# gmarcais/Jellyfish

Measured on AMD Instinct MI355X. Metric: k-mers/sec at k=21 canonical, 150 bp synthetic reads, bit-exact counts, higher is better.
Workload: dtype u64

## Files before the change

include/jfgpu.h:

```cpp
#ifndef JFGPU_H
#define JFGPU_H
#include <stddef.h>
#include <stdint.h>

#ifdef __cplusplus
extern "C" {
#endif

#define JFGPU_ABI_VERSION 1

enum {
  JFGPU_OK = 0,
  JFGPU_E_INVALID = 1,
  JFGPU_E_NO_DEVICE = 2,
  JFGPU_E_ALLOC = 3,
  JFGPU_E_FULL = 4,
  JFGPU_E_HIP = 5,
  JFGPU_E_UNSUPPORTED = 6,
  JFGPU_E_FORMAT = 7,
  JFGPU_E_CORRUPT = 8
};

typedef struct jfgpu_table jfgpu_table;

// ... 16 lines not shown
  uint32_t k, key_len;
  uint32_t canonical;
  uint32_t lsize;
  uint64_t size;
  uint64_t local_size;
  uint32_t shard_bits, shard_id;
  uint32_t val_len;
  uint32_t slot_bytes;
  uint32_t tile_slots;
  uint32_t matrix_identity;
  uint32_t out_counter_len;
  uint32_t max_reprobe;
  uint64_t table_bytes;
} jfgpu_info;

typedef struct jfgpu_stats {
  uint64_t unique;
  uint64_t distinct;
  uint64_t total;
  uint64_t max_count;
  uint64_t occupied;
  uint64_t mers_fed;
} jfgpu_stats;

const char* jfgpu_last_error(void);
int  jfgpu_abi_version(void);
int  jfgpu_device_count(void);

int  jfgpu_create(const jfgpu_params* params, jfgpu_table** out);
void jfgpu_destroy(jfgpu_table* t);
int  jfgpu_get_info(const jfgpu_table* t, jfgpu_info* out);
int  jfgpu_get_matrix(const jfgpu_table* t, uint64_t* columns );
int  jfgpu_clear(jfgpu_table* t);
int  jfgpu_sync(jfgpu_table* t);
int  jfgpu_wait(jfgpu_table* t);

int  jfgpu_count_ascii_dev(jfgpu_table* t, const char* d_bases, size_t n);
int  jfgpu_count_ascii(jfgpu_table* t, const char* bases, size_t n);

int  jfgpu_add_keys_dev(jfgpu_table* t, const uint64_t* d_keys, size_t n, uint64_t val, uint8_t* d_is_new);
int  jfgpu_add_keys(jfgpu_table* t, const uint64_t* keys, size_t n, uint64_t val, uint8_t* is_new);

int  jfgpu_add_key_vals(jfgpu_table* t, const uint64_t* keys, const uint64_t* vals, size_t n);

int  jfgpu_lookup_dev(jfgpu_table* t, const uint64_t* d_keys, size_t n, uint64_t* d_vals, uint8_t* d_found);
int  jfgpu_lookup(jfgpu_table* t, const uint64_t* keys, size_t n, uint64_t* vals, uint8_t* found);

int  jfgpu_partition_ascii_dev(jfgpu_table* t, const char* d_bases, size_t n,
                               uint64_t* d_keys_out, size_t capacity, uint64_t* counts_out);

typedef struct jfgpu_comm jfgpu_comm;
int  jfgpu_comm_unique_id(uint8_t* id128);
int  jfgpu_comm_create(int world, int rank, const uint8_t* id128, int device, jfgpu_comm** out);
int  jfgpu_comm_create_local(int world, int device, jfgpu_comm** out);
void jfgpu_comm_destroy(jfgpu_comm* c);
int  jfgpu_comm_count_ascii_dev(jfgpu_comm* c, jfgpu_table* t, const char* d_bases, size_t n);
int  jfgpu_comm_local_step(jfgpu_comm* c, jfgpu_table** tables, const char* const* d_bases, const size_t* n);
int  jfgpu_comm_finish(jfgpu_comm* c, uint64_t* sent, uint64_t* received);
int  jfgpu_comm_allreduce_u64(jfgpu_comm* c, uint64_t* values, int n, int op);
int  jfgpu_comm_allgather_u64(jfgpu_comm* c, uint64_t mine, uint64_t* all);
int  jfgpu_comm_world(const jfgpu_comm* c, int* world, int* rank);
int  jfgpu_comm_exchange_times(jfgpu_comm* c, double* ms, uint64_t* wire_bytes, size_t cap, size_t* n);

int  jfgpu_stats_compute(jfgpu_table* t, uint64_t lower, uint64_t upper, jfgpu_stats* out);
int  jfgpu_digest(jfgpu_table* t, uint64_t lower, uint64_t upper, uint64_t* out4);
int  jfgpu_histo(jfgpu_table* t, uint64_t base, uint64_t ceil, uint64_t inc, uint64_t* histo, uint64_t nb_buckets);
int  jfgpu_dump_begin(jfgpu_table* t, uint64_t lower, uint64_t upper, uint64_t* n_records, uint32_t* record_bytes);
int  jfgpu_dump_next(jfgpu_table* t, void* out, uint64_t capacity_records, uint64_t* n_read);
int  jfgpu_dump_end(jfgpu_table* t);

typedef struct jfgpu_bloom jfgpu_bloom;
typedef struct jfgpu_bloom_params {
  uint32_t k, canonical;
  uint64_t m;
  uint32_t nb_hashes;
  int32_t  device;
  uint64_t seed;
  const uint64_t* matrix1;
  const uint64_t* matrix2;
} jfgpu_bloom_params;
uint64_t jfgpu_bc_opt_m(double fp, uint64_t n);
uint32_t jfgpu_bc_opt_k(double fp);
int  jfgpu_bc_create(const jfgpu_bloom_params* p, jfgpu_bloom** out);
void jfgpu_bc_destroy(jfgpu_bloom* b);
int  jfgpu_bc_insert_ascii_dev(jfgpu_bloom* b, const char* d_bases, size_t n);
int  jfgpu_bc_insert_ascii(jfgpu_bloom* b, const char* bases, size_t n);
int  jfgpu_bc_sync(jfgpu_bloom* b, uint64_t* mers_fed);
int  jfgpu_bc_clear(jfgpu_bloom* b);
int  jfgpu_bc_get_info(const jfgpu_bloom* b, uint64_t* m, uint32_t* nb_hashes, uint64_t* nb_bytes,
                       uint64_t* matrix1 , uint64_t* matrix2);
int  jfgpu_bc_read(jfgpu_bloom* b, uint8_t* out);
int  jfgpu_bc_load(jfgpu_bloom* b, const uint8_t* data);
int  jfgpu_bc_keys(jfgpu_bloom* b, const uint64_t* keys, size_t n, uint8_t* out, int do_insert);
int  jfgpu_bf_create(const jfgpu_bloom_params* p, jfgpu_bloom** out);
int  jfgpu_bc_set_mode(jfgpu_bloom* b, int mode);
int  jfgpu_bc_reserve(jfgpu_bloom* b, uint64_t workspace_bytes);
int  jfgpu_bc_profile_enable(jfgpu_bloom* b, int on);
int  jfgpu_bc_profile_get(jfgpu_bloom* b, int which, double* ms, uint64_t* launches, uint64_t* units);
int  jfgpu_bc_profile_reset(jfgpu_bloom* b);
int  jfgpu_attach_bloom(jfgpu_table* t, jfgpu_bloom* b);
int  jfgpu_comm_bc_merge(jfgpu_comm* c, jfgpu_bloom* b);
int  jfgpu_comm_bc_merge_local(jfgpu_comm* c, jfgpu_bloom** blooms);

int  jfgpu_set_growth(jfgpu_table* t, int on);

int  jfgpu_reference_matrix(uint32_t lsize, uint32_t key_len, uint64_t* columns);

#define JFGPU_OP_COUNT  0
#define JFGPU_OP_PRIME  1
#define JFGPU_OP_UPDATE 2
int  jfgpu_set_operation(jfgpu_table* t, int op);

int  jfgpu_table_bytes(uint32_t k, uint64_t size, uint64_t* slots, uint64_t* bytes);

int  jfgpu_set_spill(jfgpu_table* t, int (*fn)(void* user), void* user);

int  jfgpu_set_mode(jfgpu_table* t, int mode);
int  jfgpu_reserve(jfgpu_table* t, uint64_t input_bytes);

typedef struct jfgpu_parser jfgpu_parser;
#define JFGPU_PARSE_FASTA    1u
#define JFGPU_PARSE_FASTQ    2u
#define JFGPU_PARSE_CONTINUE 4u
int  jfgpu_parser_create(int device, uint32_t k, jfgpu_parser** out);
void jfgpu_parser_destroy(jfgpu_parser* p);
int  jfgpu_parser_parse_dev(jfgpu_parser* p, const char* d_bytes, size_t n, unsigned flags,
                            const char** d_out, size_t* n_out, uint64_t* n_records);
int  jfgpu_parser_parse(jfgpu_parser* p, const char* bytes, size_t n, unsigned flags,
                        const char** d_out, size_t* n_out, uint64_t* n_records);
int  jfgpu_parser_host_buffer(jfgpu_parser* p, int which, size_t bytes, char** out);
int  jfgpu_parser_upload(jfgpu_parser* p, int which, const char* bytes, size_t n);
int  jfgpu_parser_upload_wait(jfgpu_parser* p, int which);
int  jfgpu_parser_parse_uploaded(jfgpu_parser* p, int which, unsigned flags,
                                 const char** d_out, size_t* n_out, uint64_t* n_records);
int  jfgpu_parser_set_min_quality(jfgpu_parser* p, int min_qual_char);
int  jfgpu_parser_last_ms(jfgpu_parser* p, double* ms);

typedef struct jfgpu_bgzf_block {
  uint64_t c_off, u_off;
  uint32_t c_len, isize, crc32, reserved;
} jfgpu_bgzf_block;
int  jfgpu_bgzf_scan(const void* bytes, size_t n, jfgpu_bgzf_block* out, size_t cap, size_t* n_blocks, size_t* n_used);
int  jfgpu_parser_inflate_uploaded(jfgpu_parser* p, int which, const jfgpu_bgzf_block* blocks, size_t n_blocks,
                                   size_t* stream_len);
int  jfgpu_parser_stream_read(jfgpu_parser* p, size_t offset, size_t n, void* dst);
int  jfgpu_parser_stream_consume(jfgpu_parser* p, size_t n);
int  jfgpu_parser_bam_decode(jfgpu_parser* p, size_t skip, int32_t n_ref, const char** d_out, size_t* n_out,
                             uint64_t* n_records, size_t* n_left);

int  jfgpu_profile_enable(jfgpu_table* t, int on);
int  jfgpu_profile_get(jfgpu_table* t, int which, double* ms, uint64_t* launches, uint64_t* units);
int  jfgpu_profile_reset(jfgpu_table* t);
int  jfgpu_profile_spans(jfgpu_table* t, int* which, double* ms, size_t cap, size_t* n);
#define JFGPU_N_COUNTERS 16
int  jfgpu_get_counters(jfgpu_table* t, uint64_t* out, uint32_t n);
int  jfgpu_gen_reads_dev(jfgpu_table* t, char* d_out, uint64_t first_read, uint64_t n_reads, uint32_t read_len, uint64_t seed);
int  jfgpu_gen_genome_reads_dev(jfgpu_table* t, char* d_out, uint64_t first_read, uint64_t n_reads, uint32_t read_len,
                                uint64_t genome_len, double substitution_rate, uint64_t seed);
int  jfgpu_gups(jfgpu_table* t, uint64_t n_updates, int mode, double* updates_per_s);
int  jfgpu_malloc_host(size_t bytes, void** out);
int  jfgpu_free_host(void* p);
int  jfgpu_malloc_dev(jfgpu_table* t, size_t bytes, void** out);
int  jfgpu_free_dev(jfgpu_table* t, void* p);
int  jfgpu_memcpy_h2d(jfgpu_table* t, void* d_dst, const void* src, size_t bytes);
int  jfgpu_memcpy_d2h(jfgpu_table* t, void* dst, const void* d_src, size_t bytes);

#ifdef __cplusplus
}
#endif
#endif
```

jellyfish_amd/capi.py:

```python
import ctypes as C
import os

import numpy as np

_HERE = os.path.dirname(os.path.abspath(__file__))
LIB_PATH = os.environ.get("JFGPU_LIB") or os.path.join(_HERE, "lib", "libjfgpu.so")

OK, E_INVALID, E_NO_DEVICE, E_ALLOC, E_FULL, E_HIP, E_UNSUPPORTED, E_FORMAT, E_CORRUPT = range(9)
PARSE_FASTA, PARSE_FASTQ, PARSE_CONTINUE = 1, 2, 4


class JfgpuError(RuntimeError):
    def __init__(self, code, msg):
        super().__init__(f"jfgpu error {code}: {msg}")
        self.code = code
        self.msg = msg


class Params(C.Structure):
    _fields_ = [
        ("k", C.c_uint32), ("canonical", C.c_uint32), ("size", C.c_uint64), ("device", C.c_int32),
        ("shard_bits", C.c_uint32), ("shard_id", C.c_uint32), ("matrix_seed", C.c_uint64),
        ("matrix_columns", C.POINTER(C.c_uint64)), ("out_counter_len", C.c_uint32), ("matrix_kind", C.c_uint32),
    ]
# ... 213 lines not shown
    def matrix_is_xorshift(self):
        cols = self.matrix()
        r, c = int(self.info.lsize), int(self.info.key_len)
        if c > 128 or r >= c or r >= 64:
            return False
        img = lambda j: xs_hash(1 << j, r, c) if c <= 64 else (xs_hash_wide(1 << j, 0, r) if j < 64 else xs_hash_wide(0, 1 << (j - 64), r))
        return all(int(cols[c - 1 - j]) == img(j) for j in range(c))

    def close(self):
        if getattr(self, "_h", None):
            self._lib.jfgpu_destroy(self._h)
            self._h = None

    __del__ = close

    def __enter__(self):
        return self

    def __exit__(self, *a):
        self.close()

    def matrix(self):
        cols = np.zeros(2 * self.k, dtype=np.uint64)
        _check(self._lib.jfgpu_get_matrix(self._h, cols.ctypes.data))
        return cols

    def clear(self):
        _check(self._lib.jfgpu_clear(self._h))

    def sync(self):
        _check(self._lib.jfgpu_sync(self._h))
        _check(self._lib.jfgpu_get_info(self._h, C.byref(self.info)))

    def wait(self):
        _check(self._lib.jfgpu_wait(self._h))

    def count_ascii(self, bases: bytes):
        buf = np.frombuffer(bases, dtype=np.uint8)
        _check(self._lib.jfgpu_count_ascii(self._h, buf.ctypes.data if len(bases) else None, len(bases)))

    def count_ascii_dev(self, d_ptr, n):
        _check(self._lib.jfgpu_count_ascii_dev(self._h, _ptr(d_ptr), n))

    def add_keys(self, keys, val=1, want_new=False):
        keys = np.ascontiguousarray(keys, dtype=np.uint64).reshape(-1, self.key_words)
        is_new = np.zeros(len(keys), dtype=np.uint8) if want_new else None
        _check(self._lib.jfgpu_add_keys(self._h, keys.ctypes.data, len(keys), val, _ptr(is_new)))
        return is_new

    def add_key_vals(self, keys, vals):
        keys = np.ascontiguousarray(keys, dtype=np.uint64).reshape(-1, self.key_words)
        vals = np.ascontiguousarray(vals, dtype=np.uint64)
        assert len(keys) == len(vals)
        _check(self._lib.jfgpu_add_key_vals(self._h, keys.ctypes.data, vals.ctypes.data, len(keys)))

    def add_keys_dev(self, d_keys, n, val=1, d_is_new=None):
        _check(self._lib.jfgpu_add_keys_dev(self._h, _ptr(d_keys), n, val, _ptr(d_is_new)))

    def lookup(self, keys):
        keys = np.ascontiguousarray(keys, dtype=np.uint64).reshape(-1, self.key_words)
        vals = np.zeros(len(keys), dtype=np.uint64)
        found = np.zeros(len(keys), dtype=np.uint8)
        _check(self._lib.jfgpu_lookup(self._h, keys.ctypes.data, len(keys), vals.ctypes.data, found.ctypes.data))
        return vals, found.astype(bool)

    def partition_ascii_dev(self, d_bases, n, d_keys_out, capacity):
        counts = np.zeros(1 << self.info.shard_bits, dtype=np.uint64)
        _check(self._lib.jfgpu_partition_ascii_dev(self._h, _ptr(d_bases), n, _ptr(d_keys_out), capacity, counts.ctypes.data))
        return counts

    def stats(self, lower=0, upper=2 ** 64 - 1):
        s = Stats()
        _check(self._lib.jfgpu_stats_compute(self._h, lower, upper, C.byref(s)))
        return s

    def digest(self, lower=0, upper=2 ** 64 - 1):
        out = np.zeros(4, dtype=np.uint64)
        _check(self._lib.jfgpu_digest(self._h, lower, upper, out.ctypes.data))
        return tuple(int(x) for x in out)

    def histo(self, low=1, high=10000, inc=1):
        base = 0 if inc >= low else low - inc
        ceil = high + inc
        nb = (ceil + inc - base) // inc
        h = np.zeros(nb, dtype=np.uint64)
        _check(self._lib.jfgpu_histo(self._h, base, ceil, inc, h.ctypes.data, nb))
        return base, inc, h

    def dump_records(self, lower=0, upper=2 ** 64 - 1, chunk_records=1 << 20):
        n = C.c_uint64()
        rb = C.c_uint32()
        _check(self._lib.jfgpu_dump_begin(self._h, lower, upper, C.byref(n), C.byref(rb)))
        try:
            chunk_records = max(chunk_records, self.info.tile_slots)
            out = np.zeros((n.value, rb.value), dtype=np.uint8)
            buf = np.zeros((chunk_records, rb.value), dtype=np.uint8)
            got = 0
            while True:
                nr = C.c_uint64()
                _check(self._lib.jfgpu_dump_next(self._h, buf.ctypes.data, chunk_records, C.byref(nr)))
                if nr.value == 0:
                    break
                out[got:got + nr.value] = buf[:nr.value]
                got += nr.value
            assert got == n.value, (got, n.value)
            return out
        finally:
            _check(self._lib.jfgpu_dump_end(self._h))

    def attach_bloom(self, bloom):
        self._bloom = bloom
        _check(self._lib.jfgpu_attach_bloom(self._h, bloom._h if bloom is not None else None))

    def set_growth(self, on):
        _check(self._lib.jfgpu_set_growth(self._h, int(bool(on))))

    def set_spill(self, fn):
        self._spill_cb = C.CFUNCTYPE(C.c_int, C.c_void_p)(lambda _u: int(fn() or 0)) if fn is not None else None
        _check(self._lib.jfgpu_set_spill(self._h, C.cast(self._spill_cb, C.c_void_p) if self._spill_cb else None, None))

    def refresh_info(self):
        _check(self._lib.jfgpu_get_info(self._h, C.byref(self.info)))
        return self.info

    def set_operation(self, op):
        _check(self._lib.jfgpu_set_operation(self._h, op))

    def set_mode(self, mode):
        _check(self._lib.jfgpu_set_mode(self._h, mode))

    def reserve(self, input_bytes):
        _check(self._lib.jfgpu_reserve(self._h, int(input_bytes)))

    def profile_enable(self, on=True):
        _check(self._lib.jfgpu_profile_enable(self._h, int(on)))

    def profile_get(self, which):
        ms, ln, un = C.c_double(), C.c_uint64(), C.c_uint64()
        _check(self._lib.jfgpu_profile_get(self._h, which, C.byref(ms), C.byref(ln), C.byref(un)))
        return ms.value, ln.value, un.value

    def profile_reset(self):
        _check(self._lib.jfgpu_profile_reset(self._h))

    def profile_spans(self, cap=65536):
        which = np.zeros(cap, dtype=np.int32)
        ms = np.zeros(cap, dtype=np.float64)
        n = C.c_size_t()
        _check(self._lib.jfgpu_profile_spans(self._h, which.ctypes.data, ms.ctypes.data, cap, C.byref(n)))
        k = min(n.value, cap)
        return list(zip(which[:k].tolist(), ms[:k].tolist()))

    COUNTER_NAMES = ("full", "mers", "ovf_full", "ovf_used", "misrouted", "direct", "t_items", "t_queued", "flushes_plain", "flushes_heavy",
                     "p2_roles", "p2_ring", "p2_sort", "p2_exact", "p1_ring", "p1_other")

    def counters(self):
        out = (C.c_uint64 * len(self.COUNTER_NAMES))()
        _check(self._lib.jfgpu_get_counters(self._h, out, len(self.COUNTER_NAMES)))
        return dict(zip(self.COUNTER_NAMES, (int(x) for x in out)))

    def gen_reads_dev(self, d_out, first_read, n_reads, read_len, seed):
        _check(self._lib.jfgpu_gen_reads_dev(self._h, _ptr(d_out), first_read, n_reads, read_len, seed))

    def gen_genome_reads_dev(self, d_out, first_read, n_reads, read_len, genome_len, substitution_rate, seed):
        _check(self._lib.jfgpu_gen_genome_reads_dev(self._h, _ptr(d_out), first_read, n_reads, read_len, genome_len, substitution_rate, seed))

    def gups(self, n_updates, mode=0):
        v = C.c_double()
        _check(self._lib.jfgpu_gups(self._h, n_updates, mode, C.byref(v)))
        return v.value

    def malloc(self, nbytes):
        p = _P()
        _check(self._lib.jfgpu_malloc_dev(self._h, nbytes, C.byref(p)))
        return p.value

    def free(self, p):
        _check(self._lib.jfgpu_free_dev(self._h, p))

    def h2d(self, d_dst, src: np.ndarray):
        src = np.ascontiguousarray(src)
        _check(self._lib.jfgpu_memcpy_h2d(self._h, d_dst, src.ctypes.data, src.nbytes))

    def d2h(self, d_src, nbytes):
        out = np.zeros(nbytes, dtype=np.uint8)
        _check(self._lib.jfgpu_memcpy_d2h(self._h, out.ctypes.data, d_src, nbytes))
        return out


def comm_unique_id():
    buf = np.zeros(128, dtype=np.uint8)
    _check(load().jfgpu_comm_unique_id(buf.ctypes.data))
    return bytes(buf)


class Comm:

    def __init__(self, world, rank=0, unique_id=None, device=-1, local=False):
        self._lib = load()
        self.world, self.rank, self.local = world, rank, local
        h = _P()
        if local:
            _check(self._lib.jfgpu_comm_create_local(world, device, C.byref(h)))
        else:
            idb = np.frombuffer(unique_id, dtype=np.uint8).copy()
            assert len(idb) == 128
            _check(self._lib.jfgpu_comm_create(world, rank, idb.ctypes.data, device, C.byref(h)))
        self._h = h

    def close(self):
        if getattr(self, "_h", None):
            self._lib.jfgpu_comm_destroy(self._h)
            self._h = None

    __del__ = close

    def step(self, table, d_ptr, n):
        _check(self._lib.jfgpu_comm_count_ascii_dev(self._h, table._h, _ptr(d_ptr), n))

    def local_step(self, tables, d_ptrs, ns):
        w = self.world
        th = (_P * w)(*[t._h for t in tables])
        dp = (_P * w)(*[_ptr(p) for p in d_ptrs])
        nn = (C.c_size_t * w)(*ns)
        _check(self._lib.jfgpu_comm_local_step(self._h, th, dp, nn))

    def finish(self):
        s, r = C.c_uint64(), C.c_uint64()
        _check(self._lib.jfgpu_comm_finish(self._h, C.byref(s), C.byref(r)))
        return s.value, r.value

    def allreduce(self, values, op="sum"):
        a = np.array(values, dtype=np.uint64)
        _check(self._lib.jfgpu_comm_allreduce_u64(self._h, a.ctypes.data, len(a), {"sum": 0, "max": 1}[op]))
        return a.tolist()

    def bc_merge(self, blooms):
        if self.local:
            arr = (_P * self.world)(*[b._h for b in blooms])
            _check(self._lib.jfgpu_comm_bc_merge_local(self._h, arr))
        else:
            _check(self._lib.jfgpu_comm_bc_merge(self._h, blooms._h))

    def world_rank(self):
        w, r = C.c_int(), C.c_int()
        _check(self._lib.jfgpu_comm_world(self._h, C.byref(w), C.byref(r)))
        return w.value, r.value

    def exchange_times(self, cap=65536):
        ms = np.zeros(cap, dtype=np.float64)
        by = np.zeros(cap, dtype=np.uint64)
        n = C.c_size_t()
        _check(self._lib.jfgpu_comm_exchange_times(self._h, ms.ctypes.data, by.ctypes.data, cap, C.byref(n)))
        k = min(n.value, cap)
        return list(zip(ms[:k].tolist(), by[:k].tolist()))

    def allgather(self, mine):
        a = np.zeros(self.world, dtype=np.uint64)
        _check(self._lib.jfgpu_comm_allgather_u64(self._h, int(mine), a.ctypes.data))
        return a.tolist()


class Bloom:

    def __init__(self, k, m, nb_hashes, canonical=True, device=-1, seed=0, matrix1=None, matrix2=None, one_pass_filter=False):
        self._lib = load()
        p = BloomParams()
        p.k, p.canonical, p.m, p.nb_hashes, p.device, p.seed = k, int(bool(canonical)), int(m), int(nb_hashes), device, seed
        self._m1 = self._m2 = None
        if matrix1 is not None:
            self._m1 = np.ascontiguousarray(matrix1, dtype=np.uint64)
            self._m2 = np.ascontiguousarray(matrix2, dtype=np.uint64)
            p.matrix1 = self._m1.ctypes.data_as(C.POINTER(C.c_uint64))
            p.matrix2 = self._m2.ctypes.data_as(C.POINTER(C.c_uint64))
        h = _P()
        _check((self._lib.jfgpu_bf_create if one_pass_filter else self._lib.jfgpu_bc_create)(C.byref(p), C.byref(h)))
        self._h = h
        self.k = k
        m_, nh, nbytes = C.c_uint64(), C.c_uint32(), C.c_uint64()
        self.matrix1 = np.zeros(2 * k, dtype=np.uint64)
        self.matrix2 = np.zeros(2 * k, dtype=np.uint64)
        _check(self._lib.jfgpu_bc_get_info(self._h, C.byref(m_), C.byref(nh), C.byref(nbytes), self.matrix1.ctypes.data, self.matrix2.ctypes.data))
        self.m, self.nb_hashes, self.nb_bytes = m_.value, nh.value, nbytes.value

    def close(self):
        if getattr(self, "_h", None):
            self._lib.jfgpu_bc_destroy(self._h)
            self._h = None

    __del__ = close

    def __enter__(self):
        return self

    def __exit__(self, *a):
        self.close()

    def insert_ascii(self, bases: bytes):
        buf = np.frombuffer(bases, dtype=np.uint8)
        _check(self._lib.jfgpu_bc_insert_ascii(self._h, buf.ctypes.data if len(bases) else None, len(bases)))

    def insert_ascii_dev(self, d_ptr, n):
        _check(self._lib.jfgpu_bc_insert_ascii_dev(self._h, _ptr(d_ptr), n))

    def sync(self):
        n = C.c_uint64()
        _check(self._lib.jfgpu_bc_sync(self._h, C.byref(n)))
# ... 160 lines not shown
```

jellyfish_amd/csrc/jfgpu.hip:

```cpp
#include <hip/hip_runtime.h>
#include <math.h>
#include <stdint.h>
#include <stdio.h>
#include <string.h>
#include <algorithm>
#include <memory>
#include <string>
#include <vector>

#include "../../include/jfgpu.h"
#include "gf2_matrix.hpp"
#include "tuning.hpp"
#include "kernels.hip.hpp"
#include "kernels_part.hip.hpp"
#include "kernels_tile.hip.hpp"
#include "kernels_p1ring.hip.hpp"
#include "kernels_bloom.hip.hpp"
#include "kernels_bloom_part.hip.hpp"
#include "kernels_wide.hip.hpp"
#include "kernels_wide_part.hip.hpp"
#include "kernels_nword.hip.hpp"
#include "kernels_parse.hip.hpp"
#include "kernels_bgzf.hip.hpp"

// ... 503 lines not shown

int jfgpu_device_count(void) {
  int n = 0;
  if(hipGetDeviceCount(&n) != hipSuccess) return 0;
  return n;
}

int jfgpu_create(const jfgpu_params* p, jfgpu_table** out) {
  if(!p || !out) return fail(JFGPU_E_INVALID, "null argument");
  *out = nullptr;
  if(p->k < 1) return fail(JFGPU_E_INVALID, "mer length must be >= 1");
  if(p->k > 128) return fail(JFGPU_E_UNSUPPORTED, "mer length > 128 (more than four key words) is not built");
  if(p->shard_bits > 8) return fail(JFGPU_E_INVALID, "at most 256 shards");
  if(p->shard_id >= (1u << p->shard_bits)) return fail(JFGPU_E_INVALID, "shard_id out of range");
  int ndev = 0;
  if(hipGetDeviceCount(&ndev) != hipSuccess || ndev == 0)
    return fail(JFGPU_E_NO_DEVICE, "no HIP device: the engine has no CPU fallback");
  int dev = p->device;
  if(dev < 0) HIP_TRY(hipGetDevice(&dev));
  if(dev >= ndev) return fail(JFGPU_E_NO_DEVICE, "device ordinal out of range");
  HIP_TRY(hipSetDevice(dev));

  const bool nword = p->k > 64, wide = p->k > 32 && !nword;
  uint32_t lsize = 0;
  while(lsize < 63 && (1ull << lsize) < p->size) ++lsize;
  if(nword) {
    lsize = std::max(lsize, nword_min_lsize(p->k));
    lsize = std::max<uint32_t>(lsize, kNTileBits + p->shard_bits);
    lsize = std::min<uint32_t>(lsize, 48);
  } else if(wide) {
    lsize = std::max(lsize, wide_min_lsize(p->k));
    lsize = std::max<uint32_t>(lsize, kMaxTileBits + p->shard_bits);
    lsize = std::min<uint32_t>(lsize, 48);
  } else {
    lsize = std::max(lsize, geom_min_lsize(p->k, p->shard_bits));
    lsize = std::max(lsize, p->shard_bits);
    lsize = std::max<uint32_t>(lsize, 1);
    lsize = std::min<uint32_t>(lsize, 2 * p->k);
    if(lsize < p->shard_bits) return fail(JFGPU_E_INVALID, "more shards than 4^k table positions");
  }

  std::unique_ptr<jfgpu_table> t(new jfgpu_table);
  t->tun = Tuning::from_env();
  t->tun.p2_cap = t->tun.p2_cap / kGran * kGran;
  t->params = *p; t->params.matrix_columns = nullptr;
  t->device = dev;
  t->out_counter_len = p->out_counter_len ? p->out_counter_len : 4;
  if(t->out_counter_len > 8) return fail(JFGPU_E_INVALID, "out_counter_len must be <= 8");
  t->wide = wide; t->nword = nword; t->key_words = (2 * p->k + 63) / 64; t->slot_words = nword ? kNWords : wide ? 2 : 1;
  if(nword) {
    if(!nword_geom_init(t->nt.N, p->k, lsize, p->canonical ? 1 : 0, p->shard_bits, p->shard_id)) return fail(JFGPU_E_INVALID, "table geometry does not fit a 256-bit slot");
    t->g = t->nt.N.g;
  } else if(wide) {
    if(!wide_geom_init(t->wt.W, p->k, lsize, p->canonical ? 1 : 0, p->shard_bits, p->shard_id)) return fail(JFGPU_E_INVALID, "table geometry does not fit a 128-bit slot");
    t->g = t->wt.W.g;
  } else if(!geom_init(t->g, p->k, lsize, p->shard_bits, p->shard_id, p->canonical ? 1 : 0, !t->tun.slot64))
    return fail(JFGPU_E_INVALID, "table geometry does not fit a 64-bit slot");

  if(p->matrix_columns) {
    t->matrix.r = lsize; t->matrix.c = 2 * p->k;
    t->matrix.columns.assign(p->matrix_columns, p->matrix_columns + 2 * p->k);
    t->matrix.identity = gf2_is_low_identity(t->matrix);
  } else if(p->matrix_seed) {
    t->matrix = gf2_random(lsize, 2 * p->k, p->matrix_seed);
  } else if(p->k <= 64 && lsize < 2 * p->k && (p->matrix_kind ? p->matrix_kind : (uint32_t)t->tun.matrix) == JFGPU_MATRIX_XORSHIFT) {
    t->xs_matrix = true;
    t->matrix = gf2_xorshift_matrix(lsize, 2 * p->k);
  } else {
    t->ref_matrix = true;
    t->matrix = lsize >= 2 * p->k ? gf2_identity(lsize, 2 * p->k) : gf2_reference_matrix(lsize, 2 * p->k, t->glibc);
  }
  if(!nword) {
    t->g.hash_xs = gf2_is_xorshift(t->matrix) ? 1 : 0;
    if(wide) t->wt.W.g.hash_xs = t->g.hash_xs;
  }
  std::vector<uint64_t> fwd, inv;
  while(!gf2_build_tables(t->matrix, fwd, inv)) {
    if(!t->ref_matrix || t->matrix.identity) return fail(JFGPU_E_INVALID, "hash matrix: low r x r block is singular");
    t->matrix = gf2_reference_matrix(lsize, 2 * p->k, t->glibc);
  }

  hipDeviceProp_t prop;
  HIP_TRY(hipGetDeviceProperties(&prop, dev));
  t->n_cu = prop.multiProcessorCount > 0 ? prop.multiProcessorCount : 256;
  HIP_TRY(hipStreamCreateWithFlags(&t->stream, hipStreamNonBlocking));

  const uint64_t n_slots = 1ull << t->g.lsize_l;
  t->ovf_cap = std::max<uint64_t>(kMinOvf, std::min<uint64_t>(n_slots / 256, 1ull << 26));
  { uint64_t c = 1; while(c < t->ovf_cap) c <<= 1; t->ovf_cap = c; }
  t->returning = t->g.cnt_bits < 40;

  DevTable& d = t->dt;
  d.g = t->g;
  HIP_TRY(hipMalloc((void**)&d.slots, n_slots * slot_bytes_of(t.get())));
  HIP_TRY(hipMalloc((void**)&t->d_fwd, fwd.size() * sizeof(uint64_t)));
  HIP_TRY(hipMalloc((void**)&t->d_inv, inv.size() * sizeof(uint64_t)));
  HIP_TRY(hipMalloc((void**)&d.ovf_key, t->ovf_cap * sizeof(uint64_t)));
  HIP_TRY(hipMalloc((void**)&d.ovf_cnt, t->ovf_cap * sizeof(uint64_t)));
  HIP_TRY(hipMalloc((void**)&d.counters, CTR_COUNT * sizeof(uint64_t)));
  HIP_TRY(hipMalloc((void**)&d.dirty, (size_t)1 << (t->g.lsize_l - t->g.tile_bits)));
  d.fwd_tbl = t->d_fwd; d.inv_tbl = t->d_inv; d.ovf_mask = t->ovf_cap - 1;
  d.max_probe = (uint32_t)std::min<uint64_t>(t->g.tile_mask, 1023);
  HIP_TRY(hipMemcpy(t->d_fwd, fwd.data(), fwd.size() * sizeof(uint64_t), hipMemcpyHostToDevice));
  HIP_TRY(hipMemcpy(t->d_inv, inv.data(), inv.size() * sizeof(uint64_t), hipMemcpyHostToDevice));
  const size_t dump_lds = ((size_t)8 << t->g.tile_bits) + ((size_t)2 << t->g.tile_bits) + (size_t)t->g.nbytes * 2048;
  HIP_TRY(hipFuncSetAttribute((const void*)dump_tiles_kernel, hipFuncAttributeMaxDynamicSharedMemorySize, (int)dump_lds));
  if(nword) {
    NTable& w = t->nt;
    w.slots = d.slots; w.fwd_tbl = d.fwd_tbl; w.inv_tbl = d.inv_tbl; w.ovf_key = d.ovf_key; w.ovf_cnt = d.ovf_cnt;
    w.ovf_mask = d.ovf_mask; w.counters = d.counters; w.max_probe = d.max_probe;
    t->part_ok = false; t->mode = MODE_DIRECT;
    const int nl = (int)(((size_t)32 << kNTileBits) + ((size_t)2 << kNTileBits));
    HIP_TRY(hipFuncSetAttribute((const void*)dump_tiles_nword_kernel, hipFuncAttributeMaxDynamicSharedMemorySize, nl));
    {
      const int rl = (int)nword_route_lds(t->g.nbytes);
      HIP_TRY(hipFuncSetAttribute((const void*)partition_count_nword_kernel, hipFuncAttributeMaxDynamicSharedMemorySize, rl));
      HIP_TRY(hipFuncSetAttribute((const void*)partition_scatter_nword_kernel, hipFuncAttributeMaxDynamicSharedMemorySize, rl));
    }
  } else if(wide) {
    WideTable& w = t->wt;
    w.slots = d.slots; w.fwd_tbl = d.fwd_tbl; w.inv_tbl = d.inv_tbl; w.ovf_key = d.ovf_key; w.ovf_cnt = d.ovf_cnt;
    w.ovf_mask = d.ovf_mask; w.counters = d.counters; w.max_probe = d.max_probe; w.dirty = d.dirty;
    memset(&w.bloom, 0, sizeof w.bloom);
    part_geom_init(t.get());
    const int wl = (int)(((size_t)16 << t->g.tile_bits) + ((size_t)2 << t->g.tile_bits));
    HIP_TRY(hipFuncSetAttribute((const void*)dump_tiles_wide_kernel, hipFuncAttributeMaxDynamicSharedMemorySize, wl));
  } else part_geom_init(t.get());
  if(!nword) {
    if(t->tun.mode == 1) t->mode = MODE_DIRECT;
    else if(t->tun.mode == 2 && t->part_ok) t->mode = MODE_PARTITIONED;
  }
  {
#define TATTR1(I, R, S, P, H, M) HIP_TRY(hipFuncSetAttribute((const void*)tile_rank_insert_kernel<I, R, S, P, kTileBlock, H, M>, hipFuncAttributeMaxDynamicSharedMemorySize, (int)tile_rank_lds(sizeof(S), kMaxTileBits, P)))
#define TATTR(I, S, P) TATTR1(I, true, S, P, false, false); TATTR1(I, false, S, P, false, false); TATTR1(I, true, S, P, true, false); TATTR1(I, false, S, P, true, false); \
                       TATTR1(I, true, S, P, false, true); TATTR1(I, false, S, P, false, true)
    TATTR(uint32_t, unsigned int, 1); TATTR(uint32_t, unsigned int, 2); TATTR(uint32_t, unsigned long long, 1);
    TATTR(uint64_t, unsigned int, 1); TATTR(uint64_t, unsigned int, 2); TATTR(uint64_t, unsigned long long, 1);
#undef TATTR
#undef TATTR1
    HIP_TRY(hipFuncSetAttribute((const void*)p1_scatter_sorted_kernel<true, true>, hipFuncAttributeMaxDynamicSharedMemorySize, kPTilePos * 6));
    HIP_TRY(hipFuncSetAttribute((const void*)p1_scatter_sorted_kernel<true, false>, hipFuncAttributeMaxDynamicSharedMemorySize, kPTilePos * 6));
    HIP_TRY(hipFuncSetAttribute((const void*)p1_scatter_sorted_kernel<false, true>, hipFuncAttributeMaxDynamicSharedMemorySize, kPTilePos * 6));
    HIP_TRY(hipFuncSetAttribute((const void*)p1_scatter_sorted_kernel<false, false>, hipFuncAttributeMaxDynamicSharedMemorySize, kPTilePos * 6));
#define PATTR(N) HIP_TRY(hipFuncSetAttribute((const void*)p1_keys_scatter_sorted_kernel<N>, hipFuncAttributeMaxDynamicSharedMemorySize, kPTilePos * 6)); \
                 HIP_TRY(hipFuncSetAttribute((const void*)p1_scatter_sorted_kernel<false, false, N>, hipFuncAttributeMaxDynamicSharedMemorySize, kPTilePos * 6))
    PATTR(0); PATTR(6); PATTR(7); PATTR(8);
#undef PATTR
    HIP_TRY(hipFuncSetAttribute((const void*)p1_keys_granule_kernel<true, 0>, hipFuncAttributeMaxDynamicSharedMemorySize, kPTilePos * 6));
    HIP_TRY(hipFuncSetAttribute((const void*)p1_keys_granule_kernel<false, 0>, hipFuncAttributeMaxDynamicSharedMemorySize, kPTilePos * 6));
    HIP_TRY(hipFuncSetAttribute((const void*)p1_keys_granule_kernel<false, 6>, hipFuncAttributeMaxDynamicSharedMemorySize, kPTilePos * 6));
    HIP_TRY(hipFuncSetAttribute((const void*)p1_keys_granule_kernel<false, 7>, hipFuncAttributeMaxDynamicSharedMemorySize, kPTilePos * 6));
    HIP_TRY(hipFuncSetAttribute((const void*)p1_keys_granule_kernel<false, 8>, hipFuncAttributeMaxDynamicSharedMemorySize, kPTilePos * 6));
    {
      const int rl = kGranMaxB * 128 + 128;
#define RATTR(IT, BL, N, CN) HIP_TRY(hipFuncSetAttribute((const void*)p1_ring_kernel<IT, BL, N, CN>, hipFuncAttributeMaxDynamicSharedMemorySize, rl))
      HIP_TRY(hipFuncSetAttribute((const void*)p2_ring_kernel<P2RingDirect>, hipFuncAttributeMaxDynamicSharedMemorySize, rl));
      HIP_TRY(hipFuncSetAttribute((const void*)p2_ring_roles_kernel<uint32_t, 2, P2RingDirect, 1>, hipFuncAttributeMaxDynamicSharedMemorySize, rl));
      HIP_TRY(hipFuncSetAttribute((const void*)p2_ring_roles_kernel<uint32_t, 1, P2RingDirect, 1>, hipFuncAttributeMaxDynamicSharedMemorySize, rl));
      HIP_TRY(hipFuncSetAttribute((const void*)p2_ring_roles_kernel<uint32_t, 2, P2RingDirect, 2>, hipFuncAttributeMaxDynamicSharedMemorySize, rl));
      HIP_TRY(hipFuncSetAttribute((const void*)p2_ring_roles_kernel<uint32_t, 1, P2RingDirect, 2>, hipFuncAttributeMaxDynamicSharedMemorySize, rl));
      HIP_TRY(hipFuncSetAttribute((const void*)p2_ring_roles_kernel<uint32_t, 2, P2RingDirect, 3>, hipFuncAttributeMaxDynamicSharedMemorySize, rl));
      HIP_TRY(hipFuncSetAttribute((const void*)p2_ring_roles_kernel<uint32_t, 1, P2RingDirect, 3>, hipFuncAttributeMaxDynamicSharedMemorySize, rl));
      RATTR(uint32_t, false, 6, 1); RATTR(uint32_t, false, 6, 0); RATTR(uint32_t, true, 0, 2); RATTR(uint32_t, false, 0, 2);
      RATTR(uint32_t, false, kHashXS, 1); RATTR(uint32_t, false, kHashXS, 0); RATTR(uint32_t, false, kHashXSLow, 2);
#undef RATTR
    }
    HIP_TRY(hipFuncSetAttribute((const void*)p2_scatter_sorted_kernel<uint32_t, 16>, hipFuncAttributeMaxDynamicSharedMemorySize, kPBlock * 16 * 4));
    HIP_TRY(hipFuncSetAttribute((const void*)p1_ring_kernel<uint32_t, false, 6, 1, RouteListDirect>, hipFuncAttributeMaxDynamicSharedMemorySize, (int)(kGranMaxB * 128 + 128)));
    HIP_TRY(hipFuncSetAttribute((const void*)p1_ring_kernel<uint32_t, false, 6, 0, RouteListDirect>, hipFuncAttributeMaxDynamicSharedMemorySize, (int)(kGranMaxB * 128 + 128)));
    HIP_TRY(hipFuncSetAttribute((const void*)p1_ring_kernel<uint32_t, false, 0, 2, RouteListDirect>, hipFuncAttributeMaxDynamicSharedMemorySize, (int)(kGranMaxB * 128 + 128)));
    HIP_TRY(hipFuncSetAttribute((const void*)p1_ring_kernel<uint32_t, true, 0, 2, RouteListDirect>, hipFuncAttributeMaxDynamicSharedMemorySize, (int)(kGranMaxB * 128 + 128)));
    HIP_TRY(hipFuncSetAttribute((const void*)p1_ring_kernel<uint32_t, false, kHashXS, 1, RouteListDirect>, hipFuncAttributeMaxDynamicSharedMemorySize, (int)(kGranMaxB * 128 + 128)));
    HIP_TRY(hipFuncSetAttribute((const void*)p1_ring_kernel<uint32_t, false, kHashXS, 0, RouteListDirect>, hipFuncAttributeMaxDynamicSharedMemorySize, (int)(kGranMaxB * 128 + 128)));
    HIP_TRY(hipFuncSetAttribute((const void*)p1_ring_kernel<uint32_t, false, kHashXSLow, 2, RouteListDirect>, hipFuncAttributeMaxDynamicSharedMemorySize, (int)(kGranMaxB * 128 + 128)));
#define SATTR(SW) HIP_TRY(hipFuncSetAttribute((const void*)p2_granule_kernel<uint32_t, TableDirect<true>, kP2PairPer, SW>, hipFuncAttributeMaxDynamicSharedMemorySize, kPBlock * kP2PairPer * 4)); \
                  HIP_TRY(hipFuncSetAttribute((const void*)p2_granule_kernel<uint32_t, TableDirect<false>, kP2PairPer, SW>, hipFuncAttributeMaxDynamicSharedMemorySize, kPBlock * kP2PairPer * 4))
    SATTR(1); SATTR(2); SATTR(4);
#undef SATTR
    HIP_TRY(hipFuncSetAttribute((const void*)p2_granule_kernel<uint64_t, TableDirect<true>, kP2MidPer>, hipFuncAttributeMaxDynamicSharedMemorySize, kPBlock * kP2MidPer * 8));
    HIP_TRY(hipFuncSetAttribute((const void*)p2_granule_kernel<uint64_t, TableDirect<false>, kP2MidPer>, hipFuncAttributeMaxDynamicSharedMemorySize, kPBlock * kP2MidPer * 8));
    HIP_TRY(hipFuncSetAttribute((const void*)p2_granule_kernel<uint32_t, TableDirect<true>, kP2PairPer>, hipFuncAttributeMaxDynamicSharedMemorySize, kPBlock * kP2PairPer * 4));
    HIP_TRY(hipFuncSetAttribute((const void*)p2_granule_kernel<uint32_t, TableDirect<false>, kP2PairPer>, hipFuncAttributeMaxDynamicSharedMemorySize, kPBlock * kP2PairPer * 4));
    HIP_TRY(hipFuncSetAttribute((const void*)p2_scatter_sorted_kernel<uint32_t, kP2PairPer>, hipFuncAttributeMaxDynamicSharedMemorySize, kPBlock * kP2PairPer * 4));
    HIP_TRY(hipFuncSetAttribute((const void*)p2_scatter_sorted_kernel<uint64_t, 14>, hipFuncAttributeMaxDynamicSharedMemorySize, kPBlock * 14 * 8));
    const int gl = kG64Chunk * 10;
    HIP_TRY(hipFuncSetAttribute((const void*)p1_granule64_kernel<true, true, 0>, hipFuncAttributeMaxDynamicSharedMemorySize, gl));
    HIP_TRY(hipFuncSetAttribute((const void*)p1_granule64_kernel<false, true, 0>, hipFuncAttributeMaxDynamicSharedMemorySize, gl));
    HIP_TRY(hipFuncSetAttribute((const void*)p1_granule64_kernel<true, false, 0>, hipFuncAttributeMaxDynamicSharedMemorySize, gl));
    HIP_TRY(hipFuncSetAttribute((const void*)p1_granule64_kernel<false, false, 0>, hipFuncAttributeMaxDynamicSharedMemorySize, gl));
    HIP_TRY(hipFuncSetAttribute((const void*)p1_granule64_kernel<false, false, 7>, hipFuncAttributeMaxDynamicSharedMemorySize, gl));
    HIP_TRY(hipFuncSetAttribute((const void*)p1_granule64_kernel<false, false, 8>, hipFuncAttributeMaxDynamicSharedMemorySize, gl));
    HIP_TRY(hipFuncSetAttribute((const void*)p1_granule64_kernel<false, false, kHashXS>, hipFuncAttributeMaxDynamicSharedMemorySize, gl));
    HIP_TRY(hipFuncSetAttribute((const void*)p1_granule64_kernel<true, false, kHashXS>, hipFuncAttributeMaxDynamicSharedMemorySize, gl));
    HIP_TRY(hipFuncSetAttribute((const void*)p2_granule_kernel<u128, WideDirect<true>, kP2WidePer>, hipFuncAttributeMaxDynamicSharedMemorySize, kPBlock * kP2WidePer * 16));
    HIP_TRY(hipFuncSetAttribute((const void*)p2_granule_kernel<u128, WideDirect<false>, kP2WidePer>, hipFuncAttributeMaxDynamicSharedMemorySize, kPBlock * kP2WidePer * 16));
    HIP_TRY(hipFuncSetAttribute((const void*)p2_scatter_sorted_kernel<u128, 7>, hipFuncAttributeMaxDynamicSharedMemorySize, kPBlock * 7 * 16));
    const int wl = kWideChunk * 18 + 16 * 2048, wt = 16 << kMaxTileBits;
    HIP_TRY(hipFuncSetAttribute((const void*)p1_wide_granule_kernel<true, true>, hipFuncAttributeMaxDynamicSharedMemorySize, wl));
    HIP_TRY(hipFuncSetAttribute((const void*)p1_wide_granule_kernel<true, false>, hipFuncAttributeMaxDynamicSharedMemorySize, wl));
    HIP_TRY(hipFuncSetAttribute((const void*)p1_wide_granule_kernel<false, true>, hipFuncAttributeMaxDynamicSharedMemorySize, wl));
    HIP_TRY(hipFuncSetAttribute((const void*)p1_wide_granule_kernel<false, false>, hipFuncAttributeMaxDynamicSharedMemorySize, wl));
    HIP_TRY(hipFuncSetAttribute((const void*)p1_wide_granule_kernel<true, false, true>, hipFuncAttributeMaxDynamicSharedMemorySize, wl));
    HIP_TRY(hipFuncSetAttribute((const void*)p1_wide_granule_kernel<false, false, true>, hipFuncAttributeMaxDynamicSharedMemorySize, wl));
    HIP_TRY(hipFuncSetAttribute((const void*)tile_insert_wide_kernel<true>, hipFuncAttributeMaxDynamicSharedMemorySize, wt));
    HIP_TRY(hipFuncSetAttribute((const void*)tile_insert_wide_kernel<false>, hipFuncAttributeMaxDynamicSharedMemorySize, wt));
    HIP_TRY(hipFuncSetAttribute((const void*)tile_insert_wide_pipe_kernel<true>, hipFuncAttributeMaxDynamicSharedMemorySize, wt));
    HIP_TRY(hipFuncSetAttribute((const void*)tile_insert_wide_pipe_kernel<false>, hipFuncAttributeMaxDynamicSharedMemorySize, wt));
  }
  jfgpu_table* raw = t.release();
  int rc = jfgpu_clear(raw);
  if(rc) { jfgpu_destroy(raw); return rc; }
  *out = raw;
  return JFGPU_OK;
}

void jfgpu_destroy(jfgpu_table* t) {
  if(!t) return;
  hipSetDevice(t->device);
  if(t->stream) hipStreamSynchronize(t->stream);
  prof_collect(t);
  for(auto e : t->ev_pool) hipEventDestroy(e);
  hipFree(t->dt.slots); hipFree(t->d_fwd); hipFree(t->d_inv);
  if(t->d_dt) hipFree(t->d_dt);
  hipFree(t->dt.ovf_key); hipFree(t->dt.ovf_cnt); hipFree(t->dt.counters); hipFree(t->dt.dirty);
  for(int i = 0; i < 2; ++i) { if(t->d_stage[i]) hipFree(t->d_stage[i]); if(t->stage_done[i]) hipEventDestroy(t->stage_done[i]); }
  if(t->d_dump) hipFree(t->d_dump);
  if(t->d_bcache) hipFree(t->d_bcache);
  if(t->d_tile_off) hipFree(t->d_tile_off);
  part_discard(t);
  if(t->d_M1) hipFree(t->d_M1);
  if(t->d_strag) hipFree(t->d_strag);
  if(t->d_strag2) hipFree(t->d_strag2);
  if(t->d_strag2_n) hipFree(t->d_strag2_n);
  if(t->d_strag_n) hipFree(t->d_strag_n);
  if(t->d_M2) hipFree(t->d_M2);
  if(t->ws) hipFree(t->ws);
  if(t->stream2) hipStreamDestroy(t->stream2);
  for(auto ev : t->flush_ev) if(ev) hipEventDestroy(ev);
  if(t->flush_done) hipEventDestroy(t->flush_done);
  if(t->stream) hipStreamDestroy(t->stream);
  delete t;
}

int jfgpu_get_info(const jfgpu_table* t, jfgpu_info* o) {
  if(!t || !o) return fail(JFGPU_E_INVALID, "null argument");
  memset(o, 0, sizeof(*o));
  o->k = t->g.k; o->key_len = t->g.key_bits; o->canonical = t->g.canonical;
  o->lsize = t->g.lsize_g; o->size = 1ull << t->g.lsize_g; o->local_size = 1ull << t->g.lsize_l;
  o->shard_bits = t->g.shard_bits; o->shard_id = t->g.shard_id;
  o->val_len = t->g.cnt_bits; o->slot_bytes = (uint32_t)slot_bytes_of(t); o->tile_slots = 1u << t->g.tile_bits;
  o->matrix_identity = t->matrix.identity ? 1 : 0;
  o->out_counter_len = t->out_counter_len;
  o->max_reprobe = t->dt.max_probe;
  o->table_bytes = (1ull << t->g.lsize_l) * slot_bytes_of(t);
  return JFGPU_OK;
}

int jfgpu_get_matrix(const jfgpu_table* t, uint64_t* columns) {
  if(!t || !columns) return fail(JFGPU_E_INVALID, "null argument");
  memcpy(columns, t->matrix.columns.data(), sizeof(uint64_t) * t->matrix.c);
  return JFGPU_OK;
}

int jfgpu_clear(jfgpu_table* t) {
  if(t) { t->failed = 0; t->failed_msg.clear(); }
  int rc = use(t); if(rc) return rc;
  part_discard(t);
  HIP_TRY(hipMemsetAsync(t->dt.slots, 0, (1ull << t->g.lsize_l) * slot_bytes_of(t), t->stream));
  HIP_TRY(hipMemsetAsync(t->dt.ovf_key, 0, t->ovf_cap * sizeof(uint64_t), t->stream));
  HIP_TRY(hipMemsetAsync(t->dt.ovf_cnt, 0, t->ovf_cap * sizeof(uint64_t), t->stream));
  HIP_TRY(hipMemsetAsync(t->dt.counters, 0, CTR_COUNT * sizeof(uint64_t), t->stream));
  HIP_TRY(hipMemsetAsync(t->dt.dirty, 0, (size_t)1 << (t->g.lsize_l - t->g.tile_bits), t->stream));
  HIP_TRY(hipStreamSynchronize(t->stream));
  t->pristine = true; t->occ_known = 0; t->fed_since = 0; t->direct_seen = 0; t->occ_bound = 0; t->bigval_bound = 0; t->ovf_failed_need = 0;
  t->flushes_plain = 0; t->flushes_heavy = 0;
  t->n_p2_roles = t->n_p2_ring = t->n_p2_sort = t->n_p2_exact = t->n_p1_ring = t->n_p1_other = 0;
  return JFGPU_OK;
}

int jfgpu_sync(jfgpu_table* t) {
  int rc = use(t); if(rc) return rc;
  rc = part_flush(t); if(rc) return rc;
  HIP_TRY(hipStreamSynchronize(t->stream));
#ifdef JFGPU_PHASE_PROF
  { unsigned long long c[24], z[24] = {0};
    if(hipMemcpyFromSymbol(c, HIP_SYMBOL(g_phase_prof), sizeof c) == hipSuccess) {
      fprintf(stderr, "[phase prof] P1 (ring): stage %llu  encode+hash+append %llu  (barrier) %llu  units out %llu  finish %llu\n",
              c[0], c[1], c[2], c[3], c[4]);
      fprintf(stderr, "[phase prof] P2: (barrier) %llu  load %llu  hist %llu  scan %llu  lds-scatter %llu  write-out %llu  finish %llu\n",
              c[8], c[9], c[10], c[11], c[12], c[13], c[14]);
      fprintf(stderr, "[phase prof] T: loop+offsets %llu  rank adds + fill %llu  place %llu  merge %llu  queue (wave 0's own) %llu  (its wait for the others) %llu  store %llu\n",
              c[16], c[17], c[18], c[22], c[21], c[19], c[20]);
      (void)hipMemcpyToSymbol(HIP_SYMBOL(g_phase_prof), z, sizeof z);
    } }
#endif
#ifdef JFGPU_TILE_PROF
  { uint64_t c[CTR_COUNT]; if(read_counters(t, c) == JFGPU_OK)
      fprintf(stderr, "[tile prof] wait+prefetch %llu  fill %llu  insert %llu  store %llu (shader clocks, summed over blocks)\n",
              (unsigned long long)c[CTR_PROF0], (unsigned long long)c[CTR_PROF0 + 1], (unsigned long long)c[CTR_PROF0 + 2], (unsigned long long)c[CTR_PROF0 + 3]); }
#endif
  return check_deferred(t);
}

int jfgpu_wait(jfgpu_table* t) {
  int rc = use(t); if(rc) return rc;
  HIP_TRY(hipStreamSynchronize(t->stream));
  return JFGPU_OK;
}

int jfgpu_count_ascii_dev(jfgpu_table* t, const char* d_bases, size_t n) {
  int rc = use(t); if(rc) return rc;
  if(t->g.shard_bits) return fail(JFGPU_E_INVALID, "sharded table: count through its communicator (jfgpu_comm_count_ascii_dev)");
  if(!d_bases && n) return fail(JFGPU_E_INVALID, "null buffer");
  return launch_count(t, d_bases, n);
}

int jfgpu_count_ascii(jfgpu_table* t, const char* bases, size_t n) {
  int rc = use(t); if(rc) return rc;
  if(t->g.shard_bits) return fail(JFGPU_E_INVALID, "sharded table: count through its communicator (jfgpu_comm_count_ascii_dev)");
  if(!bases && n) return fail(JFGPU_E_INVALID, "null buffer");
  if(n < t->g.k) return JFGPU_OK;
  rc = ensure_stage(t); if(rc) return rc;
  const size_t step = kStageBytes - (t->g.k - 1);
  for(size_t o = 0; o < n; o += step) {
    const size_t len = std::min(kStageBytes, n - o);
    const int b = t->stage_next; t->stage_next ^= 1;
    HIP_TRY(hipEventSynchronize(t->stage_done[b]));
    HIP_TRY(hipMemcpyAsync(t->d_stage[b], bases + o, len, hipMemcpyHostToDevice, t->stream));
    rc = launch_count(t, (const char*)t->d_stage[b], len); if(rc) return rc;
    HIP_TRY(hipEventRecord(t->stage_done[b], t->stream));
    if(o + len >= n) break;
  }
  return JFGPU_OK;
}

static int add_keys_piece(jfgpu_table* t, const uint64_t* d_keys, size_t n, uint64_t val, uint8_t* d_is_new) {
  int rc = JFGPU_OK;
  if(!n) return JFGPU_OK;
  { const bool big = t->g.cnt_bits < 64 && (val >> t->g.cnt_bits) != 0;
    rc = ensure_ovf(t, big ? 0 : (uint64_t)n * val, big ? n : 0); if(rc) return rc; }
  if(t->nword) {
    ProfScope ps(t, 1, n);
    t->pristine = false;
    hipLaunchKernelGGL(add_keys_nword_kernel, dim3(grid_for(t, (n + kBlock - 1) / kBlock)), dim3(kBlock), 0, t->stream, t->nt, d_keys, (uint64_t)n, t->key_words, val, d_is_new);
    HIP_TRY(hipGetLastError());
    return JFGPU_OK;
  }
  if(t->wide) {
    ProfScope ps(t, 1, n);
    hipLaunchKernelGGL(add_keys_wide_kernel, dim3(grid_for(t, (n + kBlock - 1) / kBlock)), dim3(kBlock), 0, t->stream, t->wt, d_keys, (uint64_t)n, val, d_is_new);
    HIP_TRY(hipGetLastError());
    return JFGPU_OK;
  }
  if(val == 1 && !d_is_new && use_partitioned(t, n * 8)) {
    const int prc = part_ingest(t, (const uint8_t*)d_keys, 0, (int64_t)n, true, n);
    if(prc >= 0) return prc;
  }
  if(d_is_new || val != 1) { rc = part_flush(t); if(rc) return rc; }
  t->pristine = false;
  const int grid = grid_for(t, (n + kBlock - 1) / kBlock);
  ProfScope ps(t, 1, n);
  if(val == 1 && !d_is_new) {
    if(t->returning) hipLaunchKernelGGL(add_keys_one_kernel<true>, dim3(grid), dim3(kBlock), 0, t->stream, t->dt, d_keys, (uint64_t)n);
    else             hipLaunchKernelGGL(add_keys_one_kernel<false>, dim3(grid), dim3(kBlock), 0, t->stream, t->dt, d_keys, (uint64_t)n);
  } else {
    hipLaunchKernelGGL(add_keys_kernel, dim3(grid), dim3(kBlock), 0, t->stream, t->dt, d_keys, (uint64_t)n, val, d_is_new);
  }
  HIP_TRY(hipGetLastError());
  return JFGPU_OK;
}

int jfgpu_add_keys_dev(jfgpu_table* t, const uint64_t* d_keys, size_t n, uint64_t val, uint8_t* d_is_new) {
  int rc = use(t); if(rc) return rc;
  if(!n) return JFGPU_OK;
  if(!d_keys) return fail(JFGPU_E_INVALID, "null keys");
  if(!capacity_managed(t)) return add_keys_piece(t, d_keys, n, val, d_is_new);
  size_t off = 0;
  while(off < n) {
    uint64_t take = 0;
    rc = ensure_capacity(t, n - off, &take); if(rc) return rc;
    rc = add_keys_piece(t, d_keys + off * t->key_words, (size_t)take, val, d_is_new ? d_is_new + off : nullptr); if(rc) return rc;
    off += (size_t)take;
  }
  return JFGPU_OK;
}

int jfgpu_add_keys(jfgpu_table* t, const uint64_t* keys, size_t n, uint64_t val, uint8_t* is_new) {
  int rc = use(t); if(rc) return rc;
  if(!n) return JFGPU_OK;
  uint64_t* d_k = nullptr; uint8_t* d_n = nullptr;
  HIP_TRY(hipMalloc((void**)&d_k, n * sizeof(uint64_t) * t->key_words));
  if(is_new && hipMalloc((void**)&d_n, n) != hipSuccess) { hipFree(d_k); return fail(JFGPU_E_ALLOC, "hipMalloc is_new"); }
  hipError_t e = hipMemcpyAsync(d_k, keys, n * sizeof(uint64_t) * t->key_words, hipMemcpyHostToDevice, t->stream);
  if(e == hipSuccess) { rc = jfgpu_add_keys_dev(t, d_k, n, val, d_n); }
  if(e == hipSuccess && !rc && is_new) e = hipMemcpyAsync(is_new, d_n, n, hipMemcpyDeviceToHost, t->stream);
  hipStreamSynchronize(t->stream);
  hipFree(d_k); if(d_n) hipFree(d_n);
  if(e != hipSuccess) return fail(JFGPU_E_HIP, hipGetErrorString(e));
  if(rc) return rc;
  return check_deferred(t);
}

int jfgpu_lookup_dev(jfgpu_table* t, const uint64_t* d_keys, size_t n, uint64_t* d_vals, uint8_t* d_found) {
  int rc = use(t); if(rc) return rc;
  rc = part_flush(t); if(rc) return rc;
  if(!n) return JFGPU_OK;
  if(!d_keys || !d_vals) return fail(JFGPU_E_INVALID, "null argument");
  uint64_t c[CTR_COUNT];
  rc = check_deferred(t, c); if(rc) return rc;
  const int grid = grid_for(t, (n + kBlock - 1) / kBlock);
  ProfScope ps(t, 3, n);
  if(t->nword) {
    hipLaunchKernelGGL(lookup_nword_kernel, dim3(grid), dim3(kBlock), 0, t->stream, t->nt, d_keys, (uint64_t)n, t->key_words, d_vals, d_found, (int)(c[CTR_OVF_USED] != 0));
    HIP_TRY(hipGetLastError());
    return JFGPU_OK;
  }
  if(t->wide) {
    hipLaunchKernelGGL(lookup_wide_kernel, dim3(grid), dim3(kBlock), 0, t->stream, t->wt, d_keys, (uint64_t)n, d_vals, d_found, (int)(c[CTR_OVF_USED] != 0));
    HIP_TRY(hipGetLastError());
    return JFGPU_OK;
  }
  hipLaunchKernelGGL(lookup_kernel, dim3(grid), dim3(kBlock), 0, t->stream, t->dt, d_keys, (uint64_t)n, d_vals, d_found,
                     (int)(c[CTR_OVF_USED] != 0));
  HIP_TRY(hipGetLastError());
  return JFGPU_OK;
}

int jfgpu_lookup(jfgpu_table* t, const uint64_t* keys, size_t n, uint64_t* vals, uint8_t* found) {
  int rc = use(t); if(rc) return rc;
  if(!n) return JFGPU_OK;
  uint64_t *d_k = nullptr, *d_v = nullptr; uint8_t* d_f = nullptr;
  HIP_TRY(hipMalloc((void**)&d_k, n * sizeof(uint64_t) * t->key_words));
  if(hipMalloc((void**)&d_v, n * sizeof(uint64_t)) != hipSuccess || hipMalloc((void**)&d_f, n) != hipSuccess) {
    hipFree(d_k); if(d_v) hipFree(d_v);
    return fail(JFGPU_E_ALLOC, "hipMalloc lookup buffers");
  }
  hipError_t e = hipMemcpyAsync(d_k, keys, n * sizeof(uint64_t) * t->key_words, hipMemcpyHostToDevice, t->stream);
  if(e == hipSuccess) rc = jfgpu_lookup_dev(t, d_k, n, d_v, d_f);
  if(e == hipSuccess && !rc) e = hipMemcpyAsync(vals, d_v, n * sizeof(uint64_t), hipMemcpyDeviceToHost, t->stream);
  if(e == hipSuccess && !rc && found) e = hipMemcpyAsync(found, d_f, n, hipMemcpyDeviceToHost, t->stream);
  hipStreamSynchronize(t->stream);
  hipFree(d_k); hipFree(d_v); hipFree(d_f);
  if(e != hipSuccess) return fail(JFGPU_E_HIP, hipGetErrorString(e));
// ... 154 lines not shown
  const uint32_t key_bytes = (t->g.key_bits + 7) / 8, rec = key_bytes + t->out_counter_len;
  if(t->dump_cap_records < nrec) {
    if(t->d_dump) hipFree(t->d_dump);
    t->d_dump = nullptr; t->dump_cap_records = 0;
    HIP_TRY(hipMalloc((void**)&t->d_dump, std::max<uint64_t>(nrec, capacity_records) * rec));
    t->dump_cap_records = std::max<uint64_t>(nrec, capacity_records);
  }
  if(t->tile_off_cap < ntile) {
    if(t->d_tile_off) hipFree(t->d_tile_off);
    t->d_tile_off = nullptr; t->tile_off_cap = 0;
    HIP_TRY(hipMalloc((void**)&t->d_tile_off, ntile * sizeof(uint64_t)));
    t->tile_off_cap = ntile;
  }
  std::vector<uint64_t> offs(ntile);
  for(uint64_t i = 0; i < ntile; ++i) offs[i] = t->dump_prefix[t0 + i] - t->dump_prefix[t0];
  HIP_TRY(hipMemcpyAsync(t->d_tile_off, offs.data(), ntile * sizeof(uint64_t), hipMemcpyHostToDevice, t->stream));
  if(t->nword) {
    const size_t nl = ((size_t)32 << t->g.tile_bits) + ((size_t)2 << t->g.tile_bits);
    hipLaunchKernelGGL(dump_tiles_nword_kernel, dim3(grid_for(t, ntile)), dim3(kBlock), nl, t->stream, t->nt, t->dump_lower, t->dump_upper,
                       t->dump_have_ovf, t0, ntile, (const uint64_t*)t->d_tile_off, t->d_dump, key_bytes, t->out_counter_len);
  } else if(t->wide) {
    const size_t wl = ((size_t)16 << t->g.tile_bits) + ((size_t)2 << t->g.tile_bits);
    hipLaunchKernelGGL(dump_tiles_wide_kernel, dim3(grid_for(t, ntile)), dim3(kBlock), wl, t->stream, t->wt, t->dump_lower, t->dump_upper,
                       t->dump_have_ovf, t0, ntile, (const uint64_t*)t->d_tile_off, t->d_dump, key_bytes, t->out_counter_len);
  } else {
  const size_t lds = ((size_t)8 << t->g.tile_bits) + ((size_t)2 << t->g.tile_bits) + (size_t)t->g.nbytes * 2048;
  hipLaunchKernelGGL(dump_tiles_kernel, dim3(grid_for(t, ntile)), dim3(kBlock), lds, t->stream, t->dt, t->dump_lower,
                     t->dump_upper, t->dump_have_ovf, t0, ntile, (const uint64_t*)t->d_tile_off, t->d_dump, key_bytes,
                     t->out_counter_len);
  }
  HIP_TRY(hipGetLastError());
  HIP_TRY(hipMemcpyAsync(out, t->d_dump, nrec * rec, hipMemcpyDeviceToHost, t->stream));
  HIP_TRY(hipStreamSynchronize(t->stream));
  t->dump_tile_cursor = t1;
  *n_read = nrec;
  return JFGPU_OK;
}

int jfgpu_dump_end(jfgpu_table* t) {
  int rc = use(t); if(rc) return rc;
  t->dump_open = false;
  t->dump_prefix.clear(); t->dump_prefix.shrink_to_fit();
  if(t->d_dump) { hipFree(t->d_dump); t->d_dump = nullptr; t->dump_cap_records = 0; }
  if(t->d_tile_off) { hipFree(t->d_tile_off); t->d_tile_off = nullptr; t->tile_off_cap = 0; }
  return JFGPU_OK;
}

int jfgpu_set_growth(jfgpu_table* t, int on) {
  int rc = use(t); if(rc) return rc;
  t->grow_on = on != 0;
  return JFGPU_OK;
}

int jfgpu_reserve(jfgpu_table* t, uint64_t input_bytes) {
  int rc = use(t); if(rc) return rc;
  if(!t->part_ok || t->mode == MODE_DIRECT) return JFGPU_OK;
  rc = part_flush(t); if(rc) return rc;
  t->reserved_input = input_bytes;
  const uint32_t nb1 = 1u << t->pg.b1, nb2 = 1u << t->pg.b2;
  const size_t pend = align_up(input_bytes * item_size(t), 256);
  const size_t strand = (size_t)nb1 * (2 * (size_t)t->n_cu) * kGran * item_size(t);
  const size_t headroom = t->pg.b2 ? (size_t)(pend * ((t->tun.p1_slack > 0 ? t->tun.p1_slack : 0.0) + 0.05)) + 2 * strand : 0;
  const size_t need = 2 * pend + headroom + (n_tiles_of(t) + 1 + nb1) * sizeof(uint64_t) +
                      (size_t)kMaxSeg * (align_up((2 * nb1 + 1) * sizeof(uint64_t), 256) + align_up(nb1 * 16, 256) + 1280) + ((size_t)1 << 20);
  size_t want = need;
  if(t->item128) {
    size_t free_b = 0, total_b = 0;
    HIP_TRY(hipMemGetInfo(&free_b, &total_b));
    const size_t avail = free_b + t->ws_cap > ((size_t)8 << 30) ? free_b + t->ws_cap - ((size_t)8 << 30) : 0;
    want = std::min(want, avail);
  }
  rc = ws_grow(t, want);
  if(rc < 0) return fail(JFGPU_E_ALLOC, "not enough device memory to reserve the partition workspace");
  if(rc) return rc;
  HIP_TRY(hipMemsetAsync(t->ws, 0, t->ws_cap, t->stream));
  if(!t->d_M1) { t->g1 = 2 * t->n_cu; HIP_TRY(hipMalloc((void**)&t->d_M1, (size_t)t->g1 * kMaxBuckets * sizeof(uint32_t))); }
  if(t->pg.b2 && !t->d_M2) HIP_TRY(hipMalloc((void**)&t->d_M2, (size_t)nb1 * 32 * nb2 * sizeof(uint32_t)));
  return JFGPU_OK;
}

int jfgpu_table_bytes(uint32_t k, uint64_t size, uint64_t* slots, uint64_t* bytes) {
  if(k < 1 || k > 128) return fail(JFGPU_E_UNSUPPORTED, "mer length must be in [1, 128]");
  uint32_t lsize = 0;
  while(lsize < 63 && (1ull << lsize) < size) ++lsize;
  const bool nword = k > 64, wide = k > 32 && !nword;
  if(nword) { lsize = std::max(lsize, nword_min_lsize(k)); lsize = std::min<uint32_t>(lsize, 48); }
  else if(wide) { lsize = std::max(lsize, wide_min_lsize(k)); lsize = std::min<uint32_t>(lsize, 48); }
  else { lsize = std::max(lsize, geom_min_lsize(k, 0)); lsize = std::max<uint32_t>(lsize, 1); lsize = std::min<uint32_t>(lsize, 2 * k); }
  const uint64_t n = 1ull << lsize;
  uint64_t ovf = std::max<uint64_t>(kMinOvf, std::min<uint64_t>(n / 256, 1ull << 26));
  { uint64_t c = 1; while(c < ovf) c <<= 1; ovf = c; }
  if(slots) *slots = n;
  TableGeom gg;
  const bool s32 = !nword && !wide && geom_init(gg, k, lsize, 0, 0, 1, !Tuning::from_env().slot64) && gg.slot32;
  if(bytes) *bytes = n * (nword ? 32 : wide ? 16 : s32 ? 4 : 8) + ovf * 16 + (n >> std::min<uint32_t>(lsize, kMaxTileBits)) + (size_t)(2 * k + 7) / 8 * 256 * 8 * 2;
  return JFGPU_OK;
}

int jfgpu_set_spill(jfgpu_table* t, int (*fn)(void*), void* user) {
  int rc = use(t); if(rc) return rc;
  t->spill_fn = fn; t->spill_user = user;
  return JFGPU_OK;
}

int jfgpu_reference_matrix(uint32_t lsize, uint32_t key_len, uint64_t* columns) {
  if(!columns || lsize < 1 || lsize > 64 || key_len < 2 || key_len > 256) return fail(JFGPU_E_INVALID, "bad matrix dimensions");
  GlibcRandom rng;
  const Gf2Matrix m = lsize >= key_len ? gf2_identity(lsize, key_len) : gf2_reference_matrix(lsize, key_len, rng);
  for(uint32_t i = 0; i < key_len; ++i) columns[i] = m.columns[i];
  return JFGPU_OK;
}

int jfgpu_set_operation(jfgpu_table* t, int op) {
  int rc = use(t); if(rc) return rc;
  if(op < 0 || op > 2) return fail(JFGPU_E_INVALID, "operation must be 0 (count), 1 (prime) or 2 (update)");
  if(op != t->operation) { rc = part_flush(t); if(rc) return rc; }
  t->operation = op;
  return JFGPU_OK;
}

int jfgpu_set_mode(jfgpu_table* t, int mode) {
  int rc = use(t); if(rc) return rc;
  if(mode < 0 || mode > 2) return fail(JFGPU_E_INVALID, "mode must be 0 (auto), 1 (direct) or 2 (partitioned)");
  if(mode == MODE_PARTITIONED && !t->part_ok) return fail(JFGPU_E_UNSUPPORTED, "table geometry has no partitioned path");
  rc = part_flush(t); if(rc) return rc;
  t->mode = mode;
  return JFGPU_OK;
}

int jfgpu_profile_enable(jfgpu_table* t, int on) {
  int rc = use(t); if(rc) return rc;
  t->prof_on = on != 0;
  return JFGPU_OK;
}

int jfgpu_profile_get(jfgpu_table* t, int which, double* ms, uint64_t* launches, uint64_t* units) {
  int rc = use(t); if(rc) return rc;
  if(which < 0 || which >= kNumProf) return fail(JFGPU_E_INVALID, "bad profile slot");
  HIP_TRY(hipStreamSynchronize(t->stream));
  prof_collect(t);
  if(ms) *ms = t->prof_ms[which];
  if(launches) *launches = t->prof_launches[which];
  if(units) *units = t->prof_units[which];
  return JFGPU_OK;
}

int jfgpu_get_counters(jfgpu_table* t, uint64_t* out, uint32_t n) {
  int rc = use(t); if(rc) return rc;
  if(!out) return fail(JFGPU_E_INVALID, "null argument");
  uint64_t c[CTR_COUNT];
  rc = read_counters(t, c); if(rc) return rc;
  const uint64_t v[JFGPU_N_COUNTERS] = {c[CTR_FULL], c[CTR_MERS], c[CTR_OVF_FULL], c[CTR_OVF_USED], c[CTR_MISROUTED], c[CTR_DIRECT],
                                        c[CTR_T_ITEMS], c[CTR_T_QUEUED], t->flushes_plain, t->flushes_heavy,
                                        t->n_p2_roles, t->n_p2_ring, t->n_p2_sort, t->n_p2_exact, t->n_p1_ring, t->n_p1_other};
  for(uint32_t i = 0; i < n; ++i) out[i] = i < JFGPU_N_COUNTERS ? v[i] : 0;
  return JFGPU_OK;
}

int jfgpu_profile_reset(jfgpu_table* t) {
  int rc = use(t); if(rc) return rc;
  HIP_TRY(hipStreamSynchronize(t->stream));
  prof_collect(t);
  for(int i = 0; i < kNumProf; ++i) { t->prof_ms[i] = 0; t->prof_launches[i] = 0; t->prof_units[i] = 0; }
  t->prof_log.clear();
  return JFGPU_OK;
}

int jfgpu_profile_spans(jfgpu_table* t, int* which, double* ms, size_t cap, size_t* n) {
  int rc = use(t); if(rc) return rc;
  if(!n) return fail(JFGPU_E_INVALID, "null argument");
  HIP_TRY(hipStreamSynchronize(t->stream));
  prof_collect(t);
  *n = t->prof_log.size();
  for(size_t i = 0; i < t->prof_log.size() && i < cap; ++i) { if(which) which[i] = t->prof_log[i].first; if(ms) ms[i] = t->prof_log[i].second; }
  return JFGPU_OK;
}

int jfgpu_gen_reads_dev(jfgpu_table* t, char* d_out, uint64_t first_read, uint64_t n_reads, uint32_t read_len, uint64_t seed) {
  int rc = use(t); if(rc) return rc;
  if(!n_reads) return JFGPU_OK;
  if(!d_out) return fail(JFGPU_E_INVALID, "null buffer");
  if(read_len < 1 || read_len > 2048) return fail(JFGPU_E_INVALID, "read_len must be in [1, 2048]");
  if(((uintptr_t)d_out & 15) != 0) return fail(JFGPU_E_INVALID, "gen_reads: output must be 16-byte aligned");
  const uint64_t vecs = (n_reads * ((uint64_t)read_len + 1) + 15) / 16;
  hipLaunchKernelGGL(gen_reads_kernel, dim3(grid_for(t, (vecs + kBlock - 1) / kBlock)), dim3(kBlock), 0, t->stream,
                     (uint8_t*)d_out, first_read, n_reads, read_len, seed);
  HIP_TRY(hipGetLastError());
  return JFGPU_OK;
}

int jfgpu_gen_genome_reads_dev(jfgpu_table* t, char* d_out, uint64_t first_read, uint64_t n_reads, uint32_t read_len,
                               uint64_t genome_len, double substitution_rate, uint64_t seed) {
  int rc = use(t); if(rc) return rc;
  if(!n_reads) return JFGPU_OK;
  if(!d_out) return fail(JFGPU_E_INVALID, "null buffer");
  if(read_len < 1 || read_len > 2048 || genome_len < read_len) return fail(JFGPU_E_INVALID, "read_len must be in [1, 2048] and <= genome_len");
  if(substitution_rate < 0 || substitution_rate > 0.5) return fail(JFGPU_E_INVALID, "substitution rate must be in [0, 0.5]");
  if(((uintptr_t)d_out & 15) != 0) return fail(JFGPU_E_INVALID, "gen_genome_reads: output must be 16-byte aligned");
  const uint64_t vecs = (n_reads * ((uint64_t)read_len + 1) + 15) / 16;
  hipLaunchKernelGGL(gen_genome_reads_kernel, dim3(grid_for(t, (vecs + kBlock - 1) / kBlock)), dim3(kBlock), 0, t->stream,
                     (uint8_t*)d_out, first_read, n_reads, read_len, genome_len, (uint32_t)lrint(substitution_rate * 65536.0), seed);
  HIP_TRY(hipGetLastError());
  return JFGPU_OK;
}

int jfgpu_gups(jfgpu_table* t, uint64_t n_updates, int mode, double* ups) {
  int rc = use(t); if(rc) return rc;
  if(!ups) return fail(JFGPU_E_INVALID, "null out");
  unsigned long long* d_sink = nullptr;
  HIP_TRY(hipMalloc((void**)&d_sink, sizeof(unsigned long long)));
  HIP_TRY(hipMemsetAsync(d_sink, 0, sizeof(unsigned long long), t->stream));
  hipEvent_t a, b;
  HIP_TRY(hipEventCreate(&a)); HIP_TRY(hipEventCreate(&b));
  const uint64_t mask = (((1ull << t->g.lsize_l) * slot_bytes_of(t)) >> 3) - 1;
  t->pristine = false;
  HIP_TRY(hipMemsetAsync(t->dt.dirty, 1, (size_t)1 << (t->g.lsize_l - t->g.tile_bits), t->stream));
  const int grid = grid_for(t, (n_updates + kBlock - 1) / kBlock);
  hipLaunchKernelGGL(gups_kernel, dim3(grid), dim3(kBlock), 0, t->stream, t->dt.slots, mask, std::min<uint64_t>(n_updates, 1u << 20), mode, 1ull, d_sink);
  HIP_TRY(hipEventRecord(a, t->stream));
  hipLaunchKernelGGL(gups_kernel, dim3(grid), dim3(kBlock), 0, t->stream, t->dt.slots, mask, n_updates, mode, 42ull, d_sink);
  HIP_TRY(hipEventRecord(b, t->stream));
  HIP_TRY(hipEventSynchronize(b));
  float ms = 0;
  HIP_TRY(hipEventElapsedTime(&ms, a, b));
  hipEventDestroy(a); hipEventDestroy(b); hipFree(d_sink);
  *ups = ms > 0 ? (double)n_updates / (ms * 1e-3) : 0;
  return JFGPU_OK;
}

int jfgpu_malloc_host(size_t bytes, void** out) {
  if(!out) return fail(JFGPU_E_INVALID, "null out");
  *out = nullptr;
  HIP_TRY(hipHostMalloc(out, bytes ? bytes : 16, hipHostMallocDefault));
  return JFGPU_OK;
}
int jfgpu_free_host(void* p) {
  if(p) HIP_TRY(hipHostFree(p));
  return JFGPU_OK;
}
int jfgpu_malloc_dev(jfgpu_table* t, size_t bytes, void** out) {
  int rc = use(t); if(rc) return rc;
  if(!out) return fail(JFGPU_E_INVALID, "null out");
  HIP_TRY(hipMalloc(out, bytes ? bytes : 16));
  return JFGPU_OK;
}
int jfgpu_free_dev(jfgpu_table* t, void* p) {
  int rc = use(t); if(rc) return rc;
  HIP_TRY(hipStreamSynchronize(t->stream));
  HIP_TRY(hipFree(p));
  return JFGPU_OK;
}
int jfgpu_memcpy_h2d(jfgpu_table* t, void* d_dst, const void* src, size_t bytes) {
  int rc = use(t); if(rc) return rc;
  HIP_TRY(hipMemcpyAsync(d_dst, src, bytes, hipMemcpyHostToDevice, t->stream));
  HIP_TRY(hipStreamSynchronize(t->stream));
  return JFGPU_OK;
}
int jfgpu_memcpy_d2h(jfgpu_table* t, void* dst, const void* d_src, size_t bytes) {
  int rc = use(t); if(rc) return rc;
  HIP_TRY(hipMemcpyAsync(dst, d_src, bytes, hipMemcpyDeviceToHost, t->stream));
  HIP_TRY(hipStreamSynchronize(t->stream));
  return JFGPU_OK;
}

}

#include "abi_bloom.inl"
#include "abi_parser.inl"
#include "abi_sam.inl"
#include "abi_comm.inl"
```

jellyfish_amd/csrc/kernels.hip.hpp:

```cpp
#pragma once
#include <hip/hip_runtime.h>
#include <stdint.h>
#include "kmer_core.hpp"

namespace jfgpu {

constexpr int kBlock = 256;
constexpr int kPerThread = kPerLane;
constexpr int kTilePos = kBlock * kPerThread;

enum Counter : int { CTR_FULL = 0, CTR_MERS = 1, CTR_OVF_FULL = 2, CTR_OVF_USED = 3, CTR_MISROUTED = 4, CTR_DIRECT = 5,
                     CTR_T_ITEMS = 6, CTR_T_QUEUED = 7 ,
                     CTR_PROF0 = 8 , CTR_COUNT = 12 };

#ifdef JFGPU_PHASE_PROF
__device__ unsigned long long g_phase_prof[24];
struct PhaseClk {
  long long acc[8] = {0, 0, 0, 0, 0, 0, 0, 0}; long long t;
  __device__ PhaseClk() { t = clock64(); }
  __device__ void mark(int i) { const long long n = clock64(); acc[i] += n - t; t = n; }
  __device__ void flush(int base) { if(threadIdx.x == 0) for(int i = 0; i < 8; ++i) if(acc[i]) atomicAdd(&g_phase_prof[base + i], (unsigned long long)acc[i]); }
};
#define JF_PHASE(pc, i) (pc).mark(i)
#define JF_PHASE_FLUSH(pc, base) (pc).flush(base)
#else
struct PhaseClk {};
#define JF_PHASE(pc, i) do {} while(0)
#define JF_PHASE_FLUSH(pc, base) do {} while(0)
#endif

struct DevBloom {
  uint32_t* data;
  uint64_t m;
  uint64_t recip;
  uint32_t nh;
  uint32_t nbytes;
  uint32_t kind;
  uint32_t pad_;
  const uint64_t* tbl1;
  const uint64_t* tbl2;
  uint64_t* cache;
  uint64_t cache_mask;
};

struct DevTable {
  TableGeom g;
  uint64_t* slots;
  const uint64_t* fwd_tbl;
  const uint64_t* inv_tbl;
  uint64_t* ovf_key;
  uint64_t* ovf_cnt;
  uint64_t ovf_mask;
  uint64_t* counters;
  uint32_t max_probe;
  DevBloom bloom;
  uint8_t* dirty;
};

#if defined(JFGPU_EMU)
__device__ __forceinline__ void lds_barrier() { __syncthreads(); }
#define JF_DYN_LDS(name) unsigned char* name = ::hip_emu::dyn_lds()
#else
__device__ __forceinline__ void lds_barrier() { asm volatile("s_waitcnt lgkmcnt(0)\n\ts_barrier" ::: "memory"); }
#define JF_DYN_LDS(name) extern __shared__ __align__(16) unsigned char name[]
#endif

__device__ inline bool bloom_admits(const DevBloom& B, uint64_t key);
__device__ inline uint32_t bloom_admit_mask(const DevBloom& B, const TableGeom& g, const LaneWords& L);

__device__ inline void ovf_add(const DevTable& T, uint64_t slot, uint64_t units) {
  const uint64_t want = slot + 1;
  uint64_t h = (slot * 0x9E3779B97F4A7C15ull) >> 20;
  for(uint64_t p = 0; p <= T.ovf_mask; ++p) {
    const uint64_t s = (h + p) & T.ovf_mask;
    unsigned long long old = atomicCAS((unsigned long long*)&T.ovf_key[s], 0ull, (unsigned long long)want);
    if(old == 0ull) atomicAdd((unsigned long long*)&T.counters[CTR_OVF_USED], 1ull);
    if(old == 0ull || old == want) {
      atomicAdd((unsigned long long*)&T.ovf_cnt[s], (unsigned long long)units);
      return;
    }
  }
  atomicAdd((unsigned long long*)&T.counters[CTR_OVF_FULL], 1ull);
}

__device__ inline uint64_t ovf_get(const DevTable& T, uint64_t slot) {
  const uint64_t want = slot + 1;
  uint64_t h = (slot * 0x9E3779B97F4A7C15ull) >> 20;
  for(uint64_t p = 0; p <= T.ovf_mask; ++p) {
    const uint64_t s = (h + p) & T.ovf_mask;
    const uint64_t k = T.ovf_key[s];
    if(k == 0) return 0;
    if(k == want) return T.ovf_cnt[s];
  }
  return 0;
}

__device__ inline uint64_t full_count(const DevTable& T, uint64_t word, uint64_t slot, bool have_ovf) {
  uint64_t c = slot_count(T.g, word);
  if(have_ovf) c += ovf_get(T, slot) << T.g.cnt_bits;
  return c;
}

__device__ __forceinline__ uint64_t slot_ld(const DevTable& T, uint64_t i) {
  return T.g.slot32 ? (uint64_t)reinterpret_cast<const uint32_t*>(T.slots)[i] : T.slots[i];
}
__device__ __forceinline__ uint64_t slot_ld_relaxed(const DevTable& T, uint64_t i) {
  if(T.g.slot32) return __hip_atomic_load(reinterpret_cast<const uint32_t*>(T.slots) + i, __ATOMIC_RELAXED, __HIP_MEMORY_SCOPE_AGENT);
  return __hip_atomic_load(&T.slots[i], __ATOMIC_RELAXED, __HIP_MEMORY_SCOPE_AGENT);
}
__device__ __forceinline__ uint64_t slot_cas(const DevTable& T, uint64_t i, uint64_t cmp, uint64_t val) {
  if(T.g.slot32) return atomicCAS(reinterpret_cast<unsigned int*>(T.slots) + i, (unsigned int)cmp, (unsigned int)val);
  return atomicCAS((unsigned long long*)&T.slots[i], (unsigned long long)cmp, (unsigned long long)val);
}
__device__ __forceinline__ uint64_t slot_add_rtn(const DevTable& T, uint64_t i, uint64_t add) {
  if(T.g.slot32) return atomicAdd(reinterpret_cast<unsigned int*>(T.slots) + i, (unsigned int)add);
  return atomicAdd((unsigned long long*)&T.slots[i], (unsigned long long)add);
}
__device__ __forceinline__ void slot_add(const DevTable& T, uint64_t i, uint64_t add) {
  if(T.g.slot32) __hip_atomic_fetch_add(reinterpret_cast<unsigned int*>(T.slots) + i, (unsigned int)add, __ATOMIC_RELAXED, __HIP_MEMORY_SCOPE_AGENT);
  else __hip_atomic_fetch_add((unsigned long long*)&T.slots[i], (unsigned long long)add, __ATOMIC_RELAXED, __HIP_MEMORY_SCOPE_AGENT);
}

template <bool RETURNING>
__device__ inline bool table_add(const DevTable& T, const uint64_t* fwd_lds, uint64_t key, uint64_t cnt) {
  const TableGeom& g = T.g;
  const uint64_t pos = hash_tables(fwd_lds, key, g.nbytes);
  const SlotAddr a = slot_addr(g, pos);
  if(a.shard != g.shard_id) {
    atomicAdd((unsigned long long*)&T.counters[CTR_MISROUTED], 1ull);
    return false;
  }
  { uint8_t* d = &T.dirty[a.tile_base >> g.tile_bits]; if(!*d) *d = 1; }
  const uint64_t tag = make_tag(g, key, a.idx0);
  const uint64_t low = g.occ_bit | tag;
  const uint64_t add = cnt << (g.tag_bits + 1);
  const uint64_t neww = add | low;
  const uint32_t tmask = (uint32_t)g.tile_mask;
  for(uint32_t p = 0; p <= T.max_probe; ++p) {
    const uint64_t slot = a.tile_base + probe_lin(a.idx0, p, tmask);
    const uint64_t old = slot_cas(T, slot, 0, neww);
    if(old == 0ull) return true;
    if((old & g.low_mask) == low) {
      if(RETURNING) {
        const uint64_t prev = slot_add_rtn(T, slot, add);
        if((prev >> (g.tag_bits + 1)) + cnt > g.cnt_max) ovf_add(T, slot, 1);
      } else {
        slot_add(T, slot, add);
      }
      return false;
    }
  }
  atomicAdd((unsigned long long*)&T.counters[CTR_FULL], 1ull);
  return false;
}

template <bool RETURNING>
__device__ inline bool table_update_add(const DevTable& T, const uint64_t* fwd_lds, uint64_t key, uint64_t cnt) {
  const TableGeom& g = T.g;
  const uint64_t pos = hash_tables(fwd_lds, key, g.nbytes);
  const SlotAddr a = slot_addr(g, pos);
  if(a.shard != g.shard_id) { atomicAdd((unsigned long long*)&T.counters[CTR_MISROUTED], 1ull); return false; }
  const uint64_t low = g.occ_bit | make_tag(g, key, a.idx0);
  const uint64_t add = cnt << (g.tag_bits + 1);
  const uint32_t tmask = (uint32_t)g.tile_mask;
  for(uint32_t p = 0; p <= T.max_probe; ++p) {
    const uint64_t slot = a.tile_base + probe_lin(a.idx0, p, tmask);
    const uint64_t old = slot_ld_relaxed(T, slot);
    if(old == 0ull) return false;
    if((old & g.low_mask) == low) {
      if(RETURNING) {
        const uint64_t prev = slot_add_rtn(T, slot, add);
        if((prev >> (g.tag_bits + 1)) + cnt > g.cnt_max) ovf_add(T, slot, 1);
      } else {
        slot_add(T, slot, add);
      }
      return true;
    }
  }
  return false;
}

// ... 514 lines not shown
```

jellyfish_amd/csrc/kernels_bloom_part.hip.hpp:

```cpp
#pragma once
#include "kernels_part.hip.hpp"
#include "kernels_p1ring.hip.hpp"
#include "kernels_bloom.hip.hpp"

namespace jfgpu {

constexpr uint32_t kBloomSegBits = 16;
constexpr uint32_t kBloomItemLow = kBloomSegBits + 3;
constexpr int kBloomPer = 10;
constexpr int kBloomChunk = kPBlock * kBloomPer;

struct BloomPart {
  uint32_t b1, b2;
  uint32_t n_seg;
  uint32_t pad_;
};

__device__ inline void bloom_item_direct(const DevBloom& B, const BloomPart& BP, uint32_t bucket, uint32_t item) {
  const uint64_t seg = ((uint64_t)bucket << BP.b2) | (item >> kBloomItemLow);
  const uint64_t byte = (seg << kBloomSegBits) | ((item >> 3) & 0xFFFFu);
  bloom_bump(B.data, byte, item & 7u);
}

struct BloomDirect {
  DevBloom B; BloomPart BP; unsigned long long* counter;
  __device__ void operator()(uint32_t bucket, uint32_t item) const { bloom_item_direct(B, BP, bucket, item); }
  __device__ unsigned long long* direct_counter() const { return counter; }
};

__device__ __attribute__((noinline)) void bloom_segment_item_direct_call(uint32_t* data, uint32_t seg, uint32_t item) {
  const uint64_t byte = ((uint64_t)seg << kBloomSegBits) | ((item >> 3) & 0xFFFFu);
  bloom_bump(data, byte, item & 7u);
}
struct BloomRingDirect {
  uint32_t* data;
  __device__ void operator()(uint32_t dest, uint64_t item, uint32_t cnt) const { for(uint32_t i = 0; i < cnt; ++i) bloom_segment_item_direct_call(data, dest, (uint32_t)item); }
};

template <int NB, int PER, bool NIB>
__device__ __forceinline__ void p1_bloom_granule_body(const DevBloom& B, const BloomPart& BP, const TableGeom& g, const uint8_t* __restrict__ base,
                                                      int64_t lo, int64_t hi, uint32_t cap,
                                                      unsigned int* __restrict__ gcur, unsigned long long* __restrict__ tot,
                                                      uint32_t* __restrict__ out, unsigned long long* __restrict__ mers) {
  constexpr int kChunk = kPBlock * PER;
  JF_DYN_LDS(s_dyn);
  uint32_t* s_item = reinterpret_cast<uint32_t*>(s_dyn);
  uint16_t* s_bkt = reinterpret_cast<uint16_t*>(s_dyn + (size_t)kChunk * 4);
  uint64_t* s_t1 = reinterpret_cast<uint64_t*>(s_dyn + (size_t)kChunk * 6);
  uint64_t* s_t2 = s_t1 + (size_t)B.nbytes * 256;
  uint4* s_tn = reinterpret_cast<uint4*>(s_dyn + (size_t)kChunk * 6);
  __shared__ uint32_t s_codes[kPBlock + 2];
  __shared__ uint32_t s_inv[kPBlock + 2];
  __shared__ GranuleLds G;
  const uint32_t nb = 1u << BP.b1;
  if constexpr(NIB) {
    for(uint32_t i = threadIdx.x; i < B.nbytes * 32; i += blockDim.x) {
      const uint32_t j = i >> 4, v = i & 15u;
      const uint32_t at = (j >> 1) * 256 + ((j & 1) ? (v << 4) : v);
      const uint64_t a = B.tbl1[at], c = B.tbl2[at];
      s_tn[i] = make_uint4((uint32_t)a, (uint32_t)(a >> 32), (uint32_t)c, (uint32_t)(c >> 32));
    }
  } else {
    load_tables_lds(s_t1, B.tbl1, B.nbytes);
    load_tables_lds(s_t2, B.tbl2, B.nbytes);
  }
  granule_init(G, nb);
  const uint32_t k = g.k;
  const uint64_t kwin = k >= 64 ? ~0ull : ((1ull << k) - 1);
  const uint32_t rc_shift = 2 * (k - 1);
  uint32_t my_mers = 0, my_direct = 0;
  const int64_t n_tiles = (hi + kPTilePos - 1) / kPTilePos;
  TileRaw R = tile_fetch(base, (int64_t)blockIdx.x * kPTilePos, lo, hi);
  for(int64_t tile = blockIdx.x; tile < n_tiles; tile += gridDim.x) {
    lds_barrier();
    const LaneWords L = tile_stage(R, tile * kPTilePos, lo, hi, s_codes, s_inv);
    R = tile_fetch(base, (tile + gridDim.x) * kPTilePos, lo, hi);
    uint64_t fw = (((uint64_t)L.p2 << 32) | L.p1) & g.key_mask;
    uint64_t rc = revcomp64(fw, k);
#pragma unroll 1
    for(int j = 0; j < kPerLane; ++j) {
      const uint64_t c = (L.cur >> (2 * (15 - j))) & 3u;
      fw = ((fw << 2) | c) & g.key_mask;
      rc = (rc >> 2) | ((3ull - c) << rc_shift);
      const bool valid = ((L.inv48 >> (15 - j)) & kwin) == 0;
      uint64_t cell = 0, inc = 0;
      if(valid) {
        ++my_mers;
        const uint64_t key = (g.canonical && rc < fw) ? rc : fw;
        if constexpr(NIB) {
          constexpr int kNibs = NB ? 2 * NB : 16;
          uint32_t a0 = 0, a1 = 0, c0 = 0, c1 = 0;
#pragma unroll
          for(int j = 0; j < kNibs; ++j)
            if(NB || (uint32_t)j < 2 * B.nbytes) { const uint4 e = s_tn[j * 16 + ((uint32_t)(key >> (4 * j)) & 15u)]; a0 ^= e.x; a1 ^= e.y; c0 ^= e.z; c1 ^= e.w; }
          cell = bloom_mod(((uint64_t)a1 << 32) | a0, B.m, B.recip);
          inc = bloom_mod(((uint64_t)c1 << 32) | c0, B.m, B.recip);
        } else {
          cell = bloom_mod(hash_tables_t<NB>(s_t1, key, B.nbytes), B.m, B.recip);
          inc = bloom_mod(hash_tables_t<NB>(s_t2, key, B.nbytes), B.m, B.recip);
        }
      }
      for(uint32_t h0 = 0; h0 < B.nh; h0 += PER) {
        lds_barrier();
        for(uint32_t q = threadIdx.x; q < nb; q += blockDim.x) G.hist[q] = 0;
        lds_barrier();
        uint32_t it[PER], dr[PER];
#pragma unroll
        for(int e = 0; e < PER; ++e) {
          dr[e] = 0xFFFFFFFFu; it[e] = 0;
          if(valid && h0 + e < B.nh) {
            uint64_t byte; uint32_t dig;
            divmod5(cell, byte, dig);
            const uint64_t seg = byte >> kBloomSegBits;
            const uint32_t b = (uint32_t)(seg >> BP.b2);
            it[e] = ((uint32_t)(seg & ((1u << BP.b2) - 1)) << kBloomItemLow) | ((uint32_t)(byte & 0xFFFFu) << 3) | dig;
            dr[e] = (b << 16) | atomicAdd(&G.hist[b], 1u);
            cell += inc; if(cell >= B.m) cell -= B.m;
          }
        }
        my_direct += granule_emit(G, nb, cap, gcur, out, s_item, s_bkt, it, dr,
                                  [&](uint32_t b, uint32_t v) { bloom_item_direct(B, BP, b, v); });
      }
    }
  }
  granule_finish(G, nb, cap, tot, out);
  uint64_t w = my_mers;
  for(int o = 32; o > 0; o >>= 1) w += __shfl_down(w, o, 64);
  if((threadIdx.x & 63) == 0 && w) atomicAdd(mers, (unsigned long long)w);
  (void)my_direct;
}

template <int NB>
__global__ __launch_bounds__(kPBlock) void p1_bloom_granule_kernel(DevBloom B, BloomPart BP, TableGeom g, const uint8_t* __restrict__ base,
                                                                   int64_t lo, int64_t hi, uint32_t cap,
                                                                   unsigned int* __restrict__ gcur, unsigned long long* __restrict__ tot,
                                                                   uint32_t* __restrict__ out, unsigned long long* __restrict__ mers) {
  p1_bloom_granule_body<NB, kBloomPer, false>(B, BP, g, base, lo, hi, cap, gcur, tot, out, mers);
}
template <int NB>
__global__ __launch_bounds__(kPBlock) __attribute__((amdgpu_waves_per_eu(8, 8)))
void p1_bloom_granule2_kernel(DevBloom B, BloomPart BP, TableGeom g, const uint8_t* __restrict__ base,
                              int64_t lo, int64_t hi, uint32_t cap,
                              unsigned int* __restrict__ gcur, unsigned long long* __restrict__ tot,
                              uint32_t* __restrict__ out, unsigned long long* __restrict__ mers) {
  p1_bloom_granule_body<NB, 5, true>(B, BP, g, base, lo, hi, cap, gcur, tot, out, mers);
}


constexpr uint32_t kBloomRingBytes = 256;
__device__ __attribute__((noinline)) void bloom_p1_item_direct_call(uint32_t* data, uint32_t b2, uint32_t bucket, uint32_t item) {
  const uint64_t seg = ((uint64_t)bucket << b2) | (item >> kBloomItemLow);
  const uint64_t byte = (seg << kBloomSegBits) | ((item >> 3) & 0xFFFFu);
  bloom_bump(data, byte, item & 7u);
}
struct BloomP1RingDirect {
  static constexpr bool kCountsDirect = false;
  uint32_t* data; uint32_t b2;
  __device__ void operator()(uint32_t bucket, uint64_t item, uint32_t cnt) const { for(uint32_t i = 0; i < cnt; ++i) bloom_p1_item_direct_call(data, b2, bucket, (uint32_t)item); }
};

template <int NB, int PER>
__global__ __launch_bounds__(kPBlock) void p1_bloom_ring_kernel(DevBloom B, BloomPart BP, TableGeom g, BloomP1RingDirect D, const uint8_t* __restrict__ base,
                                                                int64_t lo, int64_t hi, uint32_t cap,
                                                                unsigned int* __restrict__ gcur, unsigned long long* __restrict__ tot,
                                                                uint32_t* __restrict__ out, unsigned long long* __restrict__ mers,
                                                                uint64_t* __restrict__ strag, uint32_t* __restrict__ strag_n) {
  using R = Ring<uint32_t, kBloomRingBytes>;
  JF_DYN_LDS(s_dyn);
  const uint32_t nb = 1u << BP.b1;
  uint32_t* s_ring = reinterpret_cast<uint32_t*>(s_dyn);
  uint4* s_tn = reinterpret_cast<uint4*>(s_dyn + (size_t)nb * kBloomRingBytes + kBloomRingBytes);
  __shared__ uint32_t s_fill[kGranMaxB + 32];
  __shared__ uint32_t s_nstrag;
  __shared__ uint32_t s_codes[kPBlock + 2];
  __shared__ uint32_t s_inv[kPBlock + 2];
  const uint32_t t = threadIdx.x, lane = t & 63;
  const bool owner = t < nb;
  for(uint32_t i = t; i < B.nbytes * 32; i += blockDim.x) {
    const uint32_t j = i >> 4, v = i & 15u;
    const uint32_t at = (j >> 1) * 256 + ((j & 1) ? (v << 4) : v);
    const uint64_t a = B.tbl1[at], c = B.tbl2[at];
    s_tn[i] = make_uint4((uint32_t)a, (uint32_t)(a >> 32), (uint32_t)c, (uint32_t)(c >> 32));
  }
  ring_init<uint32_t, kBloomRingBytes>(s_ring, s_fill, nb, &s_nstrag);
  const uint32_t dump = nb * R::kSlots + (lane & (R::kSlots - 1));
  unsigned int* const gshort = gcur + nb;
  uint64_t* const my_strag = strag + (size_t)blockIdx.x * kStragPerBlock;
  const uint32_t k = g.k, rc_shift = 2 * (k - 1);
  const uint32_t sub_mask = (1u << BP.b2) - 1u;
  RingBooks Bk;
  if(owner) { Bk.nxt = atomicAdd(&gcur[t], kGran); Bk.nxt_asked = true; }
  uint32_t* const my_region = out + (uint64_t)t * cap;
  uint32_t my_mers = 0;
  auto straggler = [&](uint32_t b, uint32_t item, uint32_t cnt) {
    const uint32_t at = atomicAdd(&s_nstrag, 1u);
    if(at < kStragPerBlock) strag_store<uint32_t>(my_strag + at, b, item, cnt);
    else D(b, (uint64_t)item, cnt);
  };
  const int64_t n_tiles = (hi + kPTilePos - 1) / kPTilePos;
  TileRaw Rw = tile_fetch(base, (int64_t)blockIdx.x * kPTilePos, lo, hi);
  lds_barrier();
  for(int64_t tile = blockIdx.x; tile < n_tiles; tile += gridDim.x) {
    const LaneWords L = tile_stage(Rw, tile * kPTilePos, lo, hi, s_codes, s_inv);
    Rw = tile_fetch(base, (tile + gridDim.x) * kPTilePos, lo, hi);
    uint64_t fw = (((uint64_t)L.p2 << 32) | L.p1) & g.key_mask;
    uint64_t rc = revcomp64(fw, k);
    uint64_t smear = L.inv48;
    for(uint32_t s = 1; s < k; ) { const uint32_t step = s < k - s ? s : k - s; smear |= smear >> step; s += step; }
    const uint32_t vmask = ~(uint32_t)smear & 0xFFFFu;
    my_mers += (uint32_t)__popc(vmask);
#pragma unroll 1
    for(int j = 0; j < kPerLane; ++j) {
      const uint64_t c = (L.cur >> (2 * (15 - j))) & 3u;
      fw = ((fw << 2) | c) & g.key_mask;
      rc = (rc >> 2) | ((3ull - c) << rc_shift);
      const bool valid = (vmask >> (15 - j)) & 1u;
      const uint64_t key = (g.canonical && rc < fw) ? rc : fw;
      uint32_t a0 = 0, a1 = 0, c0 = 0, c1 = 0;
      constexpr int kNibs = NB ? 2 * NB : 16;
#pragma unroll
      for(int q = 0; q < kNibs; ++q)
        if(NB || (uint32_t)q < 2 * B.nbytes) { const uint4 e = s_tn[q * 16 + ((uint32_t)(key >> (4 * q)) & 15u)]; a0 ^= e.x; a1 ^= e.y; c0 ^= e.z; c1 ^= e.w; }
      uint64_t cell = bloom_mod(((uint64_t)a1 << 32) | a0, B.m, B.recip);
      const uint64_t inc = bloom_mod(((uint64_t)c1 << 32) | c0, B.m, B.recip);
      for(uint32_t h0 = 0; h0 < B.nh; h0 += PER) {
        uint32_t ea[PER], eo[PER], ei[PER];
#pragma unroll
        for(int e = 0; e < PER; ++e) {
          const bool on = valid && h0 + e < B.nh;
          uint64_t byte; uint32_t dig;
          divmod5(cell, byte, dig);
          const uint32_t seg = (uint32_t)(byte >> kBloomSegBits);
          const uint32_t b = seg >> BP.b2;
          ei[e] = ((seg & sub_mask) << kBloomItemLow) | ((uint32_t)(byte & 0xFFFFu) << 3) | dig;
          const uint32_t o = atomicAdd(&s_fill[on ? b : nb + (lane & 31u)], 1u);
          ea[e] = on ? b * R::kSlots : dump; eo[e] = on ? o : 0u;
          cell += inc; if(cell >= B.m) cell -= B.m;
        }
        uint32_t ghosts = 0;
#pragma unroll
        for(int e = 0; e < PER; ++e) {
          const uint32_t full = eo[e] & R::kFull;
          ghosts |= full;
          const uint32_t at = ea[e] + ((eo[e] + (eo[e] >> 16)) & (R::kSlots - 1));
          s_ring[full ? dump : at] = ei[e];
        }
        if(ghosts) {
#pragma unroll 1
          for(int e = 0; e < PER; ++e) if(eo[e] & R::kFull) straggler(ea[e] / R::kSlots, ei[e], 1u);
        }
        lds_barrier();
        wave_prio<3>();
        if(owner) ring_flush<uint32_t, false, kBloomRingBytes>(s_ring, s_fill, t, false, Bk, my_region, cap, gcur, gshort, straggler);
        wave_prio<0>();
#ifdef JFGPU_BLOOM_P1_BAR2
        lds_barrier();
#endif
      }
    }
  }
  lds_barrier();
  if(owner) { ring_flush<uint32_t, false, kBloomRingBytes>(s_ring, s_fill, t, true, Bk, my_region, cap, gcur, gshort, straggler); ring_finish<uint32_t>(Bk, t, my_region, cap, gshort, tot); }
  lds_barrier();
  if(t == 0) strag_n[blockIdx.x] = s_nstrag < kStragPerBlock ? s_nstrag : kStragPerBlock;
  uint64_t w = my_mers;
  for(int o = 32; o > 0; o >>= 1) w += __shfl_down(w, o, 64);
  if((threadIdx.x & 63) == 0 && w) atomicAdd(mers, (unsigned long long)w);
}

__device__ inline void bloom_lds_bump(uint32_t* s_seg, uint32_t item) {
  const uint32_t off = (item >> 3) & 0xFFFFu, dig = item & 7u;
  uint32_t* w = s_seg + (off >> 2);
  const uint32_t sh = 8 * (off & 3);
  const uint32_t add = bloom_pow3(dig) << sh;
  uint32_t old = *w;
  while(true) {
    if(bloom_digit((old >> sh) & 0xFFu, dig) >= 2) return;
    const uint32_t seen = atomicCAS(w, old, old + add);
    if(seen == old) return;
    old = seen;
  }
}

__global__ __launch_bounds__(kPBlock) void bloom_segment_kernel(DevBloom B, SegList S, uint32_t n_seg, uint32_t seg0 = 0) {
  JF_DYN_LDS(s_raw);
  uint32_t* s_seg = reinterpret_cast<uint32_t*>(s_raw);
  constexpr uint32_t kWords = (1u << kBloomSegBits) / 4;
  for(uint32_t t = blockIdx.x; t < n_seg; t += gridDim.x) {
    uint64_t n_items = 0;
    for(uint32_t s = 0; s < S.n; ++s) n_items += seg_hi(S, s, t) - seg_lo(S, s, t);
    if(n_items == 0) continue;
    uint32_t* gseg = B.data + ((size_t)seg0 + t) * kWords;
    for(uint32_t i = threadIdx.x * 4; i < kWords; i += blockDim.x * 4)
      *reinterpret_cast<uint4*>(s_seg + i) = *reinterpret_cast<const uint4*>(gseg + i);
    lds_barrier();
    for(uint32_t s = 0; s < S.n; ++s) {
      const uint64_t a = seg_lo(S, s, t), b = seg_hi(S, s, t);
      const uint32_t* src = reinterpret_cast<const uint32_t*>(S.items[s]);
      const bool holes = S.sh[s] != 0;
      constexpr int U = 8;
      for(uint64_t v0 = a + threadIdx.x; v0 < b; v0 += (uint64_t)U * blockDim.x) {
        uint32_t x[U];
#pragma unroll
        for(int u = 0; u < U; ++u) { const uint64_t v = v0 + (uint64_t)u * blockDim.x; x[u] = v < b ? src[v] : 0xFFFFFFFFu; }
#pragma unroll
        for(int u = 0; u < U; ++u) {
          const uint64_t v = v0 + (uint64_t)u * blockDim.x;
          if(v < b && !(holes && x[u] == 0xFFFFFFFFu)) bloom_lds_bump(s_seg, x[u]);
        }
      }
    }
    lds_barrier();
    for(uint32_t i = threadIdx.x * 4; i < kWords; i += blockDim.x * 4)
      *reinterpret_cast<uint4*>(gseg + i) = *reinterpret_cast<const uint4*>(s_seg + i);
    lds_barrier();
  }
}

__global__ __launch_bounds__(kBlock) void bloom_items_direct_kernel(DevBloom B, BloomPart BP, const uint32_t* __restrict__ items,
                                                                    const uint64_t* __restrict__ off, uint64_t cap) {
  const uint32_t nb = 1u << BP.b1;
  const uint64_t n = (uint64_t)nb * cap;
  for(uint64_t v = (uint64_t)blockIdx.x * blockDim.x + threadIdx.x; v < n; v += (uint64_t)gridDim.x * blockDim.x) {
    const uint32_t b = (uint32_t)(v / cap);
    if(v >= off[2 * (size_t)b + 1]) continue;
    const uint32_t it = items[v];
    if(it == 0xFFFFFFFFu) continue;
    bloom_item_direct(B, BP, b, it);
  }
}

}
```

jellyfish_amd/csrc/kernels_p1ring.hip.hpp:

```cpp
#pragma once
#include <type_traits>
#include "kernels_part.hip.hpp"

namespace jfgpu {

template <int P> __device__ __forceinline__ void wave_prio() {
#if defined(__HIP_DEVICE_COMPILE__)
  __builtin_amdgcn_s_setprio(P);
#endif
}

__device__ __forceinline__ uint32_t adm_to_vmask(uint32_t adm) {
  uint32_t r = 0;
#pragma unroll
  for(int j = 0; j < 16; ++j) r |= ((adm >> j) & 1u) << (15 - j);
  return r;
}


constexpr uint32_t kStragPerBlock = 16384;

template <typename ITEM, uint32_t RB = 128> struct Ring {
  static constexpr uint32_t kSlots = RB / sizeof(ITEM);
  static constexpr uint32_t kUnit = 64 / sizeof(ITEM);
  static constexpr uint32_t kChunk = 16 / sizeof(ITEM);
  static constexpr uint32_t kFull = 0xFFFFu & ~(kSlots - 1);
  static constexpr uint32_t kWords = sizeof(ITEM) <= 4 ? 1 : 1 + sizeof(ITEM) / 8;
  __device__ static uint32_t first_fill(uint32_t b) { return ((kChunk * b) & (kSlots - 1)) << 16; }
};

template <typename ITEM> __device__ __forceinline__ uint32_t chunk_hole_key(const uint4& v) {
  if constexpr(sizeof(ITEM) == 4) { const uint32_t a = v.x > v.y ? v.x : v.y, c = v.z > v.w ? v.z : v.w; return a > c ? a : c; }
  else if constexpr(sizeof(ITEM) == 8) { const uint32_t a = v.x & v.y, c = v.z & v.w; return a > c ? a : c; }
  else return v.x & v.y & v.z & v.w;
}
template <typename ITEM, typename F> __device__ __forceinline__ void chunk_items(const uint4& v, F&& f) {
  if constexpr(sizeof(ITEM) == 4) { f((ITEM)v.x); f((ITEM)v.y); f((ITEM)v.z); f((ITEM)v.w); }
  else if constexpr(sizeof(ITEM) == 8) { f((ITEM)(((uint64_t)v.y << 32) | v.x)); f((ITEM)(((uint64_t)v.w << 32) | v.z)); }
  else f((ITEM)(((unsigned __int128)(((uint64_t)v.w << 32) | v.z) << 64) | (((uint64_t)v.y << 32) | v.x)));
}

template <typename ITEM> __device__ __forceinline__ void strag_store(uint64_t* rec, uint32_t b, ITEM item, uint32_t cnt) {
  const uint64_t meta = ((uint64_t)(cnt < 255u ? cnt : 255u) << 56) | ((uint64_t)(b & 0xFFFFFFu) << 32);
  if constexpr(sizeof(ITEM) == 4) rec[0] = meta | (uint32_t)item;
  else if constexpr(sizeof(ITEM) == 8) { rec[0] = meta; rec[1] = (uint64_t)item; }
  else { rec[0] = meta; rec[1] = (uint64_t)item; rec[2] = (uint64_t)(item >> 64); }
}
template <typename ITEM> __device__ __forceinline__ void strag_load(const uint64_t* rec, uint32_t& b, ITEM& item, uint32_t& cnt) {
  const uint64_t meta = rec[0];
  b = (uint32_t)(meta >> 32) & 0xFFFFFFu; cnt = (uint32_t)(meta >> 56);
  if constexpr(sizeof(ITEM) == 4) item = (ITEM)(uint32_t)meta;
  else if constexpr(sizeof(ITEM) == 8) item = (ITEM)rec[1];
  else item = (ITEM)(((unsigned __int128)rec[2] << 64) | rec[1]);
}

struct RingBooks { uint32_t gpos = 0, room = 0, nxt = 0, stored = 0; bool nxt_asked = false, exhausted = false; };

template <typename ITEM, bool OWNED = false, uint32_t RB = 128, typename STRAG>
__device__ __forceinline__ void ring_flush(ITEM* s_ring, uint32_t* s_fill, uint32_t t, bool all, RingBooks& B, ITEM* my_region, uint32_t cap,
                                           unsigned int* gcur, unsigned int* gshort, STRAG&& straggler) {
  using R = Ring<ITEM, RB>;
  const ITEM hole = (ITEM)~(ITEM)0;
  const uint32_t w = s_fill[t];
  uint32_t cnt = w & 0xFFFFu; if(cnt > R::kSlots) cnt = R::kSlots;
  const uint32_t rb = (w >> 16) & (R::kSlots - 1);
  uint32_t units = cnt / R::kUnit; if(all && (cnt % R::kUnit)) ++units;
  uint32_t nout = 0;
  for(uint32_t s = 0; s < units; ++s) {
    uint4 v[4];
    const uint32_t s0 = (rb + s * R::kUnit) & (R::kSlots - 1);
#pragma unroll
    for(int q = 0; q < 4; ++q) v[q] = *reinterpret_cast<const uint4*>(s_ring + t * R::kSlots + ((s0 + R::kChunk * q) & (R::kSlots - 1)));
    if(!all) {
      uint32_t mx = 0;
#pragma unroll
      for(int q = 0; q < 4; ++q) { const uint32_t a = chunk_hole_key<ITEM>(v[q]); mx = mx > a ? mx : a; }
      if(mx == 0xFFFFFFFFu) break;
    }
    if constexpr(!OWNED) {
    if(B.room == 0 && B.nxt_asked) {
      if((uint64_t)B.nxt + kGran <= cap) { B.gpos = B.nxt; B.room = kGran; }
      else { B.exhausted = true; if(B.nxt < cap) atomicMax(&gshort[t], cap - B.nxt); }
      B.nxt_asked = false;
    }
    if(B.room == 0 && !B.exhausted) {
      const uint32_t r0 = atomicAdd(&gcur[t], kGran);
      if((uint64_t)r0 + kGran <= cap) { B.gpos = r0; B.room = kGran; }
      else { B.exhausted = true; if(r0 < cap) atomicMax(&gshort[t], cap - r0); }
    }
    }
    if(B.room) {
      uint4* dst = reinterpret_cast<uint4*>(my_region + B.gpos);
#pragma unroll
      for(int q = 0; q < 4; ++q) dst[q] = v[q];
      const uint32_t real = cnt - s * R::kUnit < R::kUnit ? cnt - s * R::kUnit : R::kUnit;
      B.gpos += R::kUnit; B.room -= R::kUnit; B.stored += real;
    } else {
#pragma unroll
      for(int q = 0; q < 4; ++q) chunk_items<ITEM>(v[q], [&](ITEM x) { if(x != hole) straggler(t, x, 1u); });
    }
#pragma unroll
    for(int q = 0; q < 4; ++q)
      *reinterpret_cast<uint4*>(s_ring + t * R::kSlots + ((s0 + R::kChunk * q) & (R::kSlots - 1))) = make_uint4(0xFFFFFFFFu, 0xFFFFFFFFu, 0xFFFFFFFFu, 0xFFFFFFFFu);
    ++nout;
  }
  if constexpr(!OWNED) { if(!all && !B.nxt_asked && !B.exhausted && B.room < R::kSlots) { B.nxt = atomicAdd(&gcur[t], kGran); B.nxt_asked = true; } }
  uint32_t expect = w;
  while(nout || (expect & 0xFFFFu) > R::kSlots) {
    uint32_t c = expect & 0xFFFFu; if(c > R::kSlots) c = R::kSlots;
    const uint32_t taken = nout * R::kUnit < c ? nout * R::kUnit : c;
    const uint32_t neww = ((((expect >> 16) + nout * R::kUnit) & 0xFFFFu) << 16) | (c - taken);
    const uint32_t old = atomicCAS(&s_fill[t], expect, neww);
    if(old == expect) break;
    expect = old;
  }
}

template <typename ITEM, uint32_t RB = 128>
__device__ __forceinline__ void ring_init(ITEM* s_ring, uint32_t* s_fill, uint32_t nb, uint32_t* s_nstrag) {
  using R = Ring<ITEM, RB>;
  for(uint32_t j = threadIdx.x; j < nb; j += blockDim.x) s_fill[j] = R::first_fill(j);
  uint4* r4 = reinterpret_cast<uint4*>(s_ring);
  for(uint32_t j = threadIdx.x; j < nb * (RB / 16) + RB / 16; j += blockDim.x) r4[j] = make_uint4(0xFFFFFFFFu, 0xFFFFFFFFu, 0xFFFFFFFFu, 0xFFFFFFFFu);
  if(threadIdx.x == 0) *s_nstrag = 0;
}

template <typename ITEM>
__device__ __forceinline__ void ring_finish(const RingBooks& B, uint32_t t, ITEM* my_region, uint32_t cap, unsigned int* gshort, unsigned long long* tot) {
  const ITEM hole = (ITEM)~(ITEM)0;
  for(uint32_t r = 0; r < B.room; ++r) my_region[B.gpos + r] = hole;
  if(B.nxt_asked) {
    if((uint64_t)B.nxt + kGran <= cap) { for(uint32_t r = 0; r < kGran; ++r) my_region[B.nxt + r] = hole; }
    else if(B.nxt < cap) atomicMax(&gshort[t], cap - B.nxt);
  }
  if(tot && B.stored) atomicAdd(&tot[t], (unsigned long long)B.stored);
}

struct OneWordDirect {
  static constexpr bool kCountsDirect = true;
  const DevTable* Tm; uint32_t b2; int returning;
  __device__ void operator()(uint32_t b, uint64_t item, uint32_t cnt) const { item_direct_call(Tm, b2, b, item, cnt, returning); }
};
struct RouteListDirect {
  static constexpr bool kCountsDirect = false;
  StragList SL;
  __device__ void operator()(uint32_t b, uint64_t item, uint32_t cnt) const {
    for(uint32_t i = 0; i < cnt; ++i) { const unsigned long long at = atomicAdd(SL.n, 1ull); if(at < SL.cap) SL.rec[at] = ((uint64_t)b << 32) | (uint32_t)item; }
  }
};

template <typename ITEM, bool BLOOM, int NB, int CANON, typename DIRECT = OneWordDirect>
__global__ __launch_bounds__(kPBlock) void p1_ring_kernel(DevTable T, DIRECT D, PartGeom P, const uint8_t* __restrict__ base,
                                                          int64_t lo, int64_t hi, uint32_t cap,
                                                          unsigned int* __restrict__ gcur,
                                                          unsigned long long* __restrict__ tot,
                                                          ITEM* __restrict__ out,
                                                          uint64_t* __restrict__ strag, uint32_t* __restrict__ strag_n) {
  using R = Ring<ITEM>;
  constexpr int RP = sizeof(ITEM) == 4 ? 8 : 4;
  JF_DYN_LDS(s_dyn);
  ITEM* s_ring = reinterpret_cast<ITEM*>(s_dyn);
  __shared__ uint64_t s_fwd[NB < 0 ? 1 : 8 * 256];
  __shared__ uint32_t s_fill[kGranMaxB + 32];
  __shared__ uint32_t s_nstrag;
  __shared__ uint32_t s_codes[kPBlock + 2];
  __shared__ uint32_t s_inv[kPBlock + 2];
  const TableGeom& g = T.g;
  const uint32_t nb = 1u << P.b1;
  const uint32_t t = threadIdx.x, lane = t & 63;
  const bool owner = t < nb;
  const ITEM hole = (ITEM)~(ITEM)0;
  if constexpr(NB >= 0) load_tables_lds(s_fwd, T.fwd_tbl, g.nbytes);
  ring_init<ITEM>(s_ring, s_fill, nb, &s_nstrag);
  const uint32_t dump = nb * R::kSlots + (lane & (R::kSlots - 1));
  [[maybe_unused]] const uint32_t xs_hi_mask = g.lsize_g > 32 ? (g.lsize_g >= 64 ? 0xFFFFFFFFu : ((1u << (g.lsize_g - 32)) - 1u)) : 0u;
  unsigned int* const gshort = gcur + nb;
  uint64_t* const my_strag = strag + (size_t)blockIdx.x * kStragPerBlock * R::kWords;
  const uint32_t k = g.k, bshift = g.lsize_l - P.b1;
  const uint32_t rc_shift = 2 * (k - 1);
  const uint32_t rest_mask = P.rest_shift >= 32 ? 0xFFFFFFFFu : ((1u << P.rest_shift) - 1u);
  RingBooks B;
  if(owner) { B.nxt = atomicAdd(&gcur[t], kGran); B.nxt_asked = true; }
  ITEM* const my_region = out + (uint64_t)t * cap;
  uint32_t my_mers = 0, my_direct = 0;

  auto straggler = [&](uint32_t b, ITEM item, uint32_t cnt) {
    const uint32_t at = atomicAdd(&s_nstrag, 1u);
    if(at < kStragPerBlock) strag_store<ITEM>(my_strag + (size_t)at * R::kWords, b, item, cnt);
    else { D(b, (uint64_t)item, cnt); ++my_direct; }
  };

  const int64_t n_tiles = (hi + kPTilePos - 1) / kPTilePos;
  TileRaw Rw = tile_fetch(base, (int64_t)blockIdx.x * kPTilePos, lo, hi);
  lds_barrier();
  [[maybe_unused]] PhaseClk pc;
  for(int64_t tile = blockIdx.x; tile < n_tiles; tile += gridDim.x) {
    const LaneWords L = tile_stage(Rw, tile * kPTilePos, lo, hi, s_codes, s_inv);
    Rw = tile_fetch(base, (tile + gridDim.x) * kPTilePos, lo, hi);
    JF_PHASE(pc, 0);
    const uint32_t adm = BLOOM ? bloom_admit_mask(T.bloom, g, L) : 0xFFFFu;
    uint64_t fw = (((uint64_t)L.p2 << 32) | L.p1) & g.key_mask;
    uint64_t rc = revcomp64(fw, k);
    uint64_t smear = L.inv48;
    for(uint32_t s = 1; s < k; ) { const uint32_t step = s < k - s ? s : k - s; smear |= smear >> step; s += step; }
    const uint32_t rawmask = ~(uint32_t)smear & 0xFFFFu;
    const uint32_t vmask = BLOOM ? (rawmask & adm_to_vmask(adm)) : rawmask;
    my_mers += (uint32_t)__popc(rawmask);
    auto rounds = [&](auto runs_tag) {
    constexpr bool RUNS = decltype(runs_tag)::value;
    uint64_t pk = 0; uint32_t pv = 0, run = 0;
#pragma unroll 1
    for(int j0 = 0; j0 < kPerLane; j0 += RP) {
      constexpr int NE = RUNS ? RP + 1 : RP;
      uint32_t ea[NE], eo[NE]; ITEM ei[NE];
      [[maybe_unused]] uint32_t spm = 0;
#pragma unroll
      for(int e = 0; e < NE; ++e) { ea[e] = dump; ei[e] = 0; eo[e] = 0; }
      auto emit = [&](int e, uint64_t key, uint32_t cnt, bool on) {
        uint32_t b; ITEM item;
        if constexpr(NB == kHashXS && sizeof(ITEM) == 4) {
          uint32_t ylo, yhi;
          xs_hash_halves<false>((uint32_t)key, (uint32_t)(key >> 32), xs_hi_mask, ylo, yhi);
          b = funnel_r(yhi, ylo, bshift) & (nb - 1);
          item = ((ylo & rest_mask) << g.rem_bits) | ((uint32_t)(key >> 32) >> (g.lsize_g - 32));
        } else {
          const uint64_t pos = NB < 0 ? xs_hash(key, g.lsize_g, g.key_bits) : hash_tables_t<(NB < 0 ? 0 : NB)>(s_fwd, key, g.nbytes);
          b = (uint32_t)(pos >> bshift) & (nb - 1);
          if constexpr(sizeof(ITEM) == 4) item = (((uint32_t)pos & rest_mask) << g.rem_bits) | (uint32_t)(key >> g.lsize_g);
          else item = make_item<ITEM>(g, P, key, pos & g.local_mask);
        }
        const bool special = on && (item == hole || cnt > 1);
        const bool normal = on && !special;
#ifndef JFGPU_P1_LATE_SPECIAL
        if(special) straggler(b, item, cnt);
        const uint32_t o = atomicAdd(&s_fill[normal ? b : nb + (lane & 31u)], 1u);
        ea[e] = normal ? b * R::kSlots : dump; ei[e] = item; eo[e] = normal ? o : 0u;
#else
        const uint32_t o = atomicAdd(&s_fill[normal ? b : nb + (lane & 31u)], 1u);
        spm |= special ? 1u << e : 0u;
        ea[e] = on ? b * R::kSlots : dump; ei[e] = item; eo[e] = normal ? o : special ? (R::kFull | ((cnt < 0xFFFFu ? cnt : 0xFFFFu) << 16)) : 0u;
#endif
      };
#ifndef JFGPU_P1_OLD_EXTRACT
      const uint32_t cur_r = L.cur << (2 * j0), ncur_r = ~cur_r, vm_r = vmask << j0;
#endif
#pragma unroll
      for(int e = 0; e < RP; ++e) {
#ifndef JFGPU_P1_OLD_EXTRACT
        const uint32_t c = (cur_r >> (2 * (15 - e))) & 3u, nc = (ncur_r >> (2 * (15 - e))) & 3u;
        const uint32_t v = vm_r & (1u << (15 - e));
#else
        const int j = j0 + e;
        const uint32_t c = (L.cur >> (2 * (15 - j))) & 3u, nc = 3u - c;
        const uint32_t v = vmask & (1u << (15 - j));
#endif
        if constexpr(NB >= 5 || NB == kHashXS) {
          const uint32_t flo = (uint32_t)fw, fhi = (uint32_t)(fw >> 32), rlo = (uint32_t)rc, rhi = (uint32_t)(rc >> 32);
          fw = ((uint64_t)(funnel_r(fhi, flo, 30) & (uint32_t)(g.key_mask >> 32)) << 32) | ((flo << 2) | c);
          rc = ((uint64_t)((rhi >> 2) | (nc << (rc_shift - 32))) << 32) | funnel_r(rhi, rlo, 2);
        } else {
          fw = ((fw << 2) | c) & g.key_mask;
          rc = (rc >> 2) | ((uint64_t)nc << rc_shift);
        }
        const uint64_t key = ((CANON == 1 || (CANON == 2 && g.canonical)) && rc < fw) ? rc : fw;
        if constexpr(RUNS) {
#ifdef JFGPU_P1_NO_RUNS
          const bool same = false;
#else
          const bool same = v && pv && key == pk;
#endif
          emit(e, pk, run, pv && !same);
          run = same ? run + 1 : 1;
          pk = key; pv = v;
        } else emit(e, key, 1u, v != 0);
      }
      if constexpr(RUNS) { if(j0 + RP >= kPerLane) { emit(NE - 1, pk, run, pv != 0); pv = 0; } }
      uint32_t ghosts = 0;
#pragma unroll
      for(int e = 0; e < NE; ++e) {
        const uint32_t full = eo[e] & R::kFull;
        ghosts |= full;
        const uint32_t at = ea[e] + ((eo[e] + (eo[e] >> 16)) & (R::kSlots - 1));
        s_ring[full ? dump : at] = ei[e];
      }
      if(ghosts) {
#pragma unroll 1
#ifndef JFGPU_P1_LATE_SPECIAL
        for(int e = 0; e < NE; ++e) {
          uint32_t a = 0, o = 0; ITEM it = 0;
#pragma unroll
          for(int q = 0; q < NE; ++q) if(q == e) { a = ea[q]; o = eo[q]; it = ei[q]; }
          if(o & R::kFull) straggler(a / R::kSlots, it, 1u);
        }
#else
        for(int e = 0; e < NE; ++e) if(eo[e] & R::kFull) straggler(ea[e] / R::kSlots, ei[e], ((spm >> e) & 1u) ? eo[e] >> 16 : 1u);
#endif
      }
      JF_PHASE(pc, 1);
      lds_barrier();
      JF_PHASE(pc, 2);
#ifndef JFGPU_P1_NO_FLUSH_PRIO
      wave_prio<3>();
#endif
      if(owner) ring_flush<ITEM>(s_ring, s_fill, t, false, B, my_region, cap, gcur, gshort, straggler);
#ifndef JFGPU_P1_NO_FLUSH_PRIO
      wave_prio<0>();
#endif
      JF_PHASE(pc, 3);
    }
    };
    bool may_run = k < 14;
    {
      const uint32_t hc = L.cur ^ (L.cur >> 2), hp = L.p1 ^ (L.p1 >> 2);
      may_run = may_run || (hc & 0x3FFFu) == 0 || ((hc >> 16) & 0x3FFFu) == 0 || (hp & 0x3FFFu) == 0;
    }
#ifdef JFGPU_P1_ALWAYS_RUNS
    may_run = true;
#endif
    if(__ballot(may_run) != 0ull) rounds(std::true_type{}); else rounds(std::false_type{});
  }
  lds_barrier();
  if(owner) { ring_flush<ITEM>(s_ring, s_fill, t, true, B, my_region, cap, gcur, gshort, straggler); ring_finish<ITEM>(B, t, my_region, cap, gshort, tot); }
  lds_barrier();
  if(t == 0) strag_n[blockIdx.x] = s_nstrag < kStragPerBlock ? s_nstrag : kStragPerBlock;
  JF_PHASE(pc, 4);
  JF_PHASE_FLUSH(pc, 0);
  if(DIRECT::kCountsDirect && my_direct) atomicAdd((unsigned long long*)&T.counters[CTR_DIRECT], (unsigned long long)my_direct);
  uint64_t w = my_mers;
  for(int o = 32; o > 0; o >>= 1) w += __shfl_down(w, o, 64);
  if((threadIdx.x & 63) == 0 && w) atomicAdd((unsigned long long*)&T.counters[CTR_MERS], (unsigned long long)w);
}

template <typename ITEM, typename DIRECT>
__global__ __launch_bounds__(256) void p1_stragglers_kernel(DIRECT D, unsigned long long* __restrict__ ctr_direct, const uint64_t* __restrict__ strag,
                                                            const uint32_t* __restrict__ strag_n, uint32_t n_lists, uint32_t cap,
                                                            unsigned int* __restrict__ gcur, unsigned long long* __restrict__ tot,
                                                            ITEM* __restrict__ out, uint32_t list_cap = kStragPerBlock) {
  using R = Ring<ITEM>;
  uint32_t my_direct = 0;
  for(uint32_t l = blockIdx.x; l < n_lists; l += gridDim.x) {
    const uint32_t n = strag_n[l];
    const uint64_t* rec = strag + (size_t)l * list_cap * R::kWords;
    for(uint32_t i = threadIdx.x; i < n; i += blockDim.x) {
      uint32_t b, cnt; ITEM item;
      strag_load<ITEM>(rec + (size_t)i * R::kWords, b, item, cnt);
      if(cnt == 1 && item != (ITEM)~(ITEM)0) {
        const uint32_t at = atomicAdd(&gcur[b], 1u);
        if(at < cap) { out[(uint64_t)b * cap + at] = item; if(tot) atomicAdd(&tot[b], 1ull); continue; }
      }
      D(b, item, cnt);
      ++my_direct;
    }
  }
  if(ctr_direct && my_direct) atomicAdd(ctr_direct, (unsigned long long)my_direct);
}

constexpr uint32_t kP2StragPerBlock = 2048;

struct P2RingDirect {
  const DevTable* Tm; uint32_t b2; uint32_t dest_shift; int returning;
  __device__ void operator()(uint32_t dest, uint64_t item, uint32_t cnt) const { item_direct_call(Tm, b2, dest >> dest_shift, item, cnt, returning); }
};

template <typename DIRECT>
__global__ __launch_bounds__(kPBlock) void p2_ring_kernel(DIRECT D, uint32_t b2e, uint32_t tag_bits, SegList S, uint32_t cap,
                                                          unsigned int* __restrict__ gcur, unsigned int* __restrict__ gshort,
                                                          uint32_t* __restrict__ out, uint32_t bucket0, unsigned long long* __restrict__ tot,
                                                          uint64_t* __restrict__ strag, uint32_t* __restrict__ strag_n, unsigned long long* __restrict__ ctr_direct) {
  using R = Ring<uint32_t>;
  constexpr int RP = 8;
  JF_DYN_LDS(s_dyn);
  uint32_t* s_ring = reinterpret_cast<uint32_t*>(s_dyn);
  __shared__ uint32_t s_fill[kGranMaxB];
  __shared__ uint32_t s_nstrag;
  const uint32_t nb = 1u << b2e;
  const uint32_t bucket = bucket0 + blockIdx.y;
  const uint32_t dest0 = bucket * nb;
  const uint32_t t = threadIdx.x, lane = t & 63;
  const bool owner = t < nb;
  const uint32_t hole = 0xFFFFFFFFu;
  ring_init<uint32_t>(s_ring, s_fill, nb, &s_nstrag);
  const uint32_t dump = nb * R::kSlots + (lane & (R::kSlots - 1));
  unsigned int* const gc = gcur + dest0;
  unsigned int* const gs = gshort + dest0;
  const uint32_t list = blockIdx.y * gridDim.x + blockIdx.x;
  uint64_t* const my_strag = strag + (size_t)list * kP2StragPerBlock;
  RingBooks B;
  if(owner) { B.nxt = atomicAdd(&gc[t], kGran); B.nxt_asked = true; }
  uint32_t* const my_region = out + ((uint64_t)dest0 + t) * cap;
  uint32_t my_direct = 0;
  auto straggler = [&](uint32_t d, uint32_t item, uint32_t cnt) {
    const uint32_t at = atomicAdd(&s_nstrag, 1u);
    if(at < kP2StragPerBlock) strag_store<uint32_t>(my_strag + at, dest0 + d, item, cnt);
    else { D(dest0 + d, (uint64_t)item, cnt); ++my_direct; }
  };
  auto flush = [&](bool all) { if(owner) ring_flush<uint32_t>(s_ring, s_fill, t, all, B, my_region, cap, gc, gs, straggler); };
  lds_barrier();
  uint32_t seg = 0; uint64_t my_a = 0, my_b = 0;
  const uint32_t* src = nullptr;
  auto next_seg = [&]() -> bool {
    for(; seg < S.n; ++seg) {
      const uint64_t a0 = seg_lo(S, seg, bucket), b0 = seg_hi(S, seg, bucket);
      const uint64_t len4 = (b0 - a0 + 3) / 4;
      const uint64_t per4 = (len4 + gridDim.x - 1) / gridDim.x;
      const uint64_t q0 = (uint64_t)blockIdx.x * per4, q1 = q0 + per4;
      const uint64_t e1 = a0 + 4 * (q1 < len4 ? q1 : len4);
      my_a = a0 + 4 * (q0 < len4 ? q0 : len4); my_b = e1 < b0 ? e1 : b0;
      src = reinterpret_cast<const uint32_t*>(S.items[seg]);
      if(my_a < my_b) return true;
    }
    return false;
  };
  constexpr uint64_t RS = (uint64_t)kPBlock * RP;
  auto load_full = [&](uint64_t r0, uint32_t (&it)[RP]) {
#pragma unroll
    for(int h = 0; h < RP / 4; ++h) {
      const uint4 v = *reinterpret_cast<const uint4*>(src + r0 + (uint64_t)h * kPBlock * 4 + 4 * (uint64_t)t);
      it[4 * h] = v.x; it[4 * h + 1] = v.y; it[4 * h + 2] = v.z; it[4 * h + 3] = v.w;
    }
  };
  auto load_partial = [&](uint64_t r0, uint32_t (&it)[RP]) {
#pragma unroll
    for(int h = 0; h < RP / 4; ++h) {
      const uint64_t i = r0 + (uint64_t)h * kPBlock * 4 + 4 * (uint64_t)t;
      uint4 v = make_uint4(hole, hole, hole, hole);
      if(i + 4 <= my_b) v = *reinterpret_cast<const uint4*>(src + i);
      else if(i < my_b) { v.x = src[i]; if(i + 1 < my_b) v.y = src[i + 1]; if(i + 2 < my_b) v.z = src[i + 2]; }
      it[4 * h] = v.x; it[4 * h + 1] = v.y; it[4 * h + 2] = v.z; it[4 * h + 3] = v.w;
    }
  };
  auto process = [&](const uint32_t (&it)[RP]) {
    uint32_t ea[RP], eo[RP];
#pragma unroll
    for(int e = 0; e < RP; ++e) {
      ea[e] = dump; eo[e] = 0;
      if(it[e] != hole) { const uint32_t d = (it[e] >> tag_bits) & (nb - 1); ea[e] = d * R::kSlots; eo[e] = atomicAdd(&s_fill[d], 1u); }
    }
    uint32_t ghosts = 0;
#pragma unroll
    for(int e = 0; e < RP; ++e) {
      const uint32_t full = eo[e] & R::kFull;
      ghosts |= full;
      const uint32_t at = ea[e] + ((eo[e] + (eo[e] >> 16)) & (R::kSlots - 1));
      s_ring[full ? dump : at] = it[e];
    }
    if(ghosts) {
#pragma unroll 1
      for(int e = 0; e < RP; ++e) if(eo[e] & R::kFull) straggler(ea[e] / R::kSlots, it[e], 1u);
    }
    lds_barrier();
    flush(false);
    lds_barrier();
  };
  for(bool have = next_seg(); have; ++seg, have = next_seg()) {
    uint64_t r0 = my_a;
    const uint64_t n_full = (my_b - my_a) / RS;
    if(n_full) {
      uint32_t nx[RP];
      load_full(r0, nx);
#pragma unroll 1
      for(uint64_t k = 0; k < n_full; ++k) {
        uint32_t it[RP];
#pragma unroll
        for(int e = 0; e < RP; ++e) it[e] = nx[e];
        r0 += RS;
        load_full(k + 1 < n_full ? r0 : my_a, nx);
        process(it);
      }
    }
    if(r0 < my_b) { uint32_t it[RP]; load_partial(r0, it); process(it); }
  }
  lds_barrier();
  flush(true);
  if(owner) ring_finish<uint32_t>(B, t, my_region, cap, gs, tot ? tot + dest0 : nullptr);
  lds_barrier();
  if(t == 0) strag_n[list] = s_nstrag < kP2StragPerBlock ? s_nstrag : kP2StragPerBlock;
  if(my_direct) atomicAdd(ctr_direct, (unsigned long long)my_direct);
}

template <typename ITEM, int NV, typename DIRECT, int PD = 1>
__global__ __launch_bounds__(kPBlock) void p2_ring_roles_kernel(DIRECT D, uint32_t b2e, uint32_t tag_bits, SegList S, uint32_t cap,
                                                                unsigned int* __restrict__ gcur, ITEM* __restrict__ out, uint32_t bucket0,
                                                                uint64_t* __restrict__ strag, uint32_t* __restrict__ strag_n, unsigned long long* __restrict__ ctr_direct) {
  using R = Ring<ITEM>;
  constexpr int VPI = (int)R::kChunk;
  constexpr int RP = NV * VPI;
  constexpr uint32_t kHalf = kPBlock / 2;
  constexpr uint64_t RS = (uint64_t)kHalf * RP;
  JF_DYN_LDS(s_dyn);
  ITEM* s_ring = reinterpret_cast<ITEM*>(s_dyn);
  __shared__ uint32_t s_fill[kGranMaxB];
  __shared__ uint32_t s_nstrag;
  const uint32_t nb = 1u << b2e;
  const uint32_t bucket = bucket0 + blockIdx.x;
  const uint32_t dest0 = bucket * nb;
  const uint32_t t = threadIdx.x, lane = t & 63;
  const bool storer = t < kHalf;
  const ITEM hole = (ITEM)~(ITEM)0;
  ring_init<ITEM>(s_ring, s_fill, nb, &s_nstrag);
  const uint32_t dump = nb * R::kSlots + (lane & (R::kSlots - 1));
  uint64_t* const my_strag = strag + (size_t)blockIdx.x * kP2StragPerBlock * R::kWords;
  uint32_t my_direct = 0;
  auto straggler = [&](uint32_t d, ITEM item, uint32_t cnt) {
    const uint32_t at = atomicAdd(&s_nstrag, 1u);
    if(at < kP2StragPerBlock) strag_store<ITEM>(my_strag + (size_t)at * R::kWords, dest0 + d, item, cnt);
    else { D(dest0 + d, item, cnt); ++my_direct; }
  };
  lds_barrier();
  auto seg_bounds = [&](uint32_t seg, uint64_t& a, uint64_t& b) { a = seg_lo(S, seg, bucket); b = seg_hi(S, seg, bucket); };
  if(storer) {
    const uint32_t d0 = t, d1 = t + kHalf;
    const bool has0 = d0 < nb, has1 = d1 < nb;
    RingBooks B0, B1;
    B0.room = B1.room = cap & ~(R::kUnit - 1);
    ITEM* const r0p = out + ((uint64_t)dest0 + d0) * cap;
    ITEM* const r1p = out + ((uint64_t)dest0 + d1) * cap;
    auto flush = [&](bool all) {
      if(has0) ring_flush<ITEM, true>(s_ring, s_fill, d0, all, B0, r0p, cap, gcur, gcur, straggler);
      if(has1) ring_flush<ITEM, true>(s_ring, s_fill, d1, all, B1, r1p, cap, gcur, gcur, straggler);
    };
    for(uint32_t seg = 0; seg < S.n; ++seg) {
      uint64_t a, b; seg_bounds(seg, a, b);
      const uint64_t rounds = (b - a + RS - 1) / RS;
#pragma unroll 1
      for(uint64_t r = 0; r < rounds; ++r) { lds_barrier(); flush(false); }
    }
    lds_barrier();
    flush(true);
    if(has0) gcur[dest0 + d0] = B0.gpos;
    if(has1) gcur[dest0 + d1] = B1.gpos;
  } else {
    const uint32_t l = t - kHalf;
    for(uint32_t seg = 0; seg < S.n; ++seg) {
      uint64_t a, b; seg_bounds(seg, a, b);
      const ITEM* src = reinterpret_cast<const ITEM*>(S.items[seg]);
      auto load_full = [&](uint64_t r0, ITEM (&it)[RP]) {
#pragma unroll
        for(int h = 0; h < NV; ++h) {
          const uint4 v = *reinterpret_cast<const uint4*>(src + r0 + (uint64_t)h * kHalf * VPI + (uint64_t)VPI * l);
          int q = 0;
          chunk_items<ITEM>(v, [&](ITEM x) { it[VPI * h + q] = x; ++q; });
        }
      };
      auto load_partial = [&](uint64_t r0, ITEM (&it)[RP]) {
#pragma unroll
        for(int h = 0; h < NV; ++h) {
          const uint64_t i = r0 + (uint64_t)h * kHalf * VPI + (uint64_t)VPI * l;
#pragma unroll
          for(int q = 0; q < VPI; ++q) it[VPI * h + q] = i + q < b ? src[i + q] : hole;
        }
      };
      auto load_exact = [&](uint64_t r0, ITEM (&it)[RP]) {
#pragma unroll 1
        for(int h = 0; h < NV; ++h) {
          const uint64_t i = r0 + (uint64_t)h * kHalf * VPI + (uint64_t)VPI * l;
#pragma unroll
          for(int q = 0; q < VPI; ++q) {
            ITEM x = hole;
            if(i + q < b) { x = src[i + q]; if(x == hole) straggler((uint32_t)(x >> tag_bits) & (nb - 1), x, 1u); }
            it[VPI * h + q] = x;
          }
        }
      };
      auto append = [&](const ITEM (&it)[RP]) {
        uint32_t ea[RP], eo[RP];
#pragma unroll
        for(int e = 0; e < RP; ++e) {
          ea[e] = dump; eo[e] = 0;
          if(it[e] != hole) { const uint32_t d = (uint32_t)(it[e] >> tag_bits) & (nb - 1); ea[e] = d * R::kSlots; eo[e] = atomicAdd(&s_fill[d], 1u); }
        }
        uint32_t ghosts = 0;
#pragma unroll
        for(int e = 0; e < RP; ++e) {
          const uint32_t full = eo[e] & R::kFull;
          ghosts |= full;
          const uint32_t at = ea[e] + ((eo[e] + (eo[e] >> 16)) & (R::kSlots - 1));
          s_ring[full ? dump : at] = it[e];
        }
        if(ghosts) {
#pragma unroll 1
          for(int e = 0; e < RP; ++e) if(eo[e] & R::kFull) straggler(ea[e] / R::kSlots, it[e], 1u);
        }
        lds_barrier();
      };
      uint64_t r0 = a;
      if(S.sh[seg] == 0) {
#pragma unroll 1
        for(; r0 < b; r0 += RS) { ITEM it[RP]; load_exact(r0, it); append(it); }
        continue;
      }
      const uint64_t n_full = (b - a) / RS;
      if(n_full) {
        ITEM nx[PD][RP];
#pragma unroll
        for(int d = 0; d < PD; ++d) load_full((uint64_t)d < n_full ? a + (uint64_t)d * RS : a, nx[d]);
        uint64_t k = 0;
#pragma unroll 1
        for(; k + PD <= n_full; k += PD) {
#pragma unroll
          for(int d = 0; d < PD; ++d) {
            ITEM it[RP];
#pragma unroll
            for(int e = 0; e < RP; ++e) it[e] = nx[d][e];
            const uint64_t nxt = k + d + PD;
            load_full(nxt < n_full ? a + nxt * RS : a, nx[d]);
            append(it);
          }
        }
#pragma unroll
        for(int d = 0; d < PD - 1; ++d)
          if(k + d < n_full) append(nx[d]);
        r0 = a + n_full * RS;
      }
      if(r0 < b) { ITEM it[RP]; load_partial(r0, it); append(it); }
    }
    lds_barrier();
  }
  lds_barrier();
  if(t == 0) strag_n[blockIdx.x] = s_nstrag < kP2StragPerBlock ? s_nstrag : kP2StragPerBlock;
  if(my_direct) atomicAdd(ctr_direct, (unsigned long long)my_direct);
}

}
```

Baseline: 15.21 billion.

## Rework LDS ring buffers to byte-offset fills, spare dump rings and peeked flush

Changes the per-destination LDS ring bookkeeping to count fills in bytes, routes hole items to a set of spare dump rings through a zero-increment atomic, and factors the store and overflow logic into shared helpers. The flush now peeks the first 64-byte unit before flushing and tracks how far the ring has been seen. It can therefore write out partially holed units instead of stopping at them, and it counts holed units and stragglers. The aim is to cut the branchy per-item dump handling and reduce stalled flushes. In exchange it adds extra atomics for holes and per-block counter updates, plus more LDS for the dump rings, and the added phase-profiling hooks are compiled out by default.

```diff
diff --git a/include/jfgpu.h b/include/jfgpu.h
--- a/include/jfgpu.h
+++ b/include/jfgpu.h
@@ -192,7 +192,7 @@
 int  jfgpu_profile_get(jfgpu_table* t, int which, double* ms, uint64_t* launches, uint64_t* units);
 int  jfgpu_profile_reset(jfgpu_table* t);
 int  jfgpu_profile_spans(jfgpu_table* t, int* which, double* ms, size_t cap, size_t* n);
-#define JFGPU_N_COUNTERS 16
+#define JFGPU_N_COUNTERS 18
 int  jfgpu_get_counters(jfgpu_table* t, uint64_t* out, uint32_t n);
 int  jfgpu_gen_reads_dev(jfgpu_table* t, char* d_out, uint64_t first_read, uint64_t n_reads, uint32_t read_len, uint64_t seed);
 int  jfgpu_gen_genome_reads_dev(jfgpu_table* t, char* d_out, uint64_t first_read, uint64_t n_reads, uint32_t read_len,
diff --git a/jellyfish_amd/capi.py b/jellyfish_amd/capi.py
--- a/jellyfish_amd/capi.py
+++ b/jellyfish_amd/capi.py
@@ -389,7 +389,7 @@
         return list(zip(which[:k].tolist(), ms[:k].tolist()))
 
     COUNTER_NAMES = ("full", "mers", "ovf_full", "ovf_used", "misrouted", "direct", "t_items", "t_queued", "flushes_plain", "flushes_heavy",
-                     "p2_roles", "p2_ring", "p2_sort", "p2_exact", "p1_ring", "p1_other")
+                     "p2_roles", "p2_ring", "p2_sort", "p2_exact", "p1_ring", "p1_other", "ring_holed_units", "ring_stragglers")
 
     def counters(self):
         out = (C.c_uint64 * len(self.COUNTER_NAMES))()
diff --git a/jellyfish_amd/csrc/jfgpu.hip b/jellyfish_amd/csrc/jfgpu.hip
--- a/jellyfish_amd/csrc/jfgpu.hip
+++ b/jellyfish_amd/csrc/jfgpu.hip
@@ -679,7 +679,7 @@
     HIP_TRY(hipFuncSetAttribute((const void*)p1_keys_granule_kernel<false, 7>, hipFuncAttributeMaxDynamicSharedMemorySize, kPTilePos * 6));
     HIP_TRY(hipFuncSetAttribute((const void*)p1_keys_granule_kernel<false, 8>, hipFuncAttributeMaxDynamicSharedMemorySize, kPTilePos * 6));
     {
-      const int rl = kGranMaxB * 128 + 128;
+      const int rl = (int)ring_lds_bytes(kGranMaxB);
 #define RATTR(IT, BL, N, CN) HIP_TRY(hipFuncSetAttribute((const void*)p1_ring_kernel<IT, BL, N, CN>, hipFuncAttributeMaxDynamicSharedMemorySize, rl))
       HIP_TRY(hipFuncSetAttribute((const void*)p2_ring_kernel<P2RingDirect>, hipFuncAttributeMaxDynamicSharedMemorySize, rl));
       HIP_TRY(hipFuncSetAttribute((const void*)p2_ring_roles_kernel<uint32_t, 2, P2RingDirect, 1>, hipFuncAttributeMaxDynamicSharedMemorySize, rl));
@@ -693,13 +693,13 @@
 #undef RATTR
     }
     HIP_TRY(hipFuncSetAttribute((const void*)p2_scatter_sorted_kernel<uint32_t, 16>, hipFuncAttributeMaxDynamicSharedMemorySize, kPBlock * 16 * 4));
-    HIP_TRY(hipFuncSetAttribute((const void*)p1_ring_kernel<uint32_t, false, 6, 1, RouteListDirect>, hipFuncAttributeMaxDynamicSharedMemorySize, (int)(kGranMaxB * 128 + 128)));
-    HIP_TRY(hipFuncSetAttribute((const void*)p1_ring_kernel<uint32_t, false, 6, 0, RouteListDirect>, hipFuncAttributeMaxDynamicSharedMemorySize, (int)(kGranMaxB * 128 + 128)));
-    HIP_TRY(hipFuncSetAttribute((const void*)p1_ring_kernel<uint32_t, false, 0, 2, RouteListDirect>, hipFuncAttributeMaxDynamicSharedMemorySize, (int)(kGranMaxB * 128 + 128)));
-    HIP_TRY(hipFuncSetAttribute((const void*)p1_ring_kernel<uint32_t, true, 0, 2, RouteListDirect>, hipFuncAttributeMaxDynamicSharedMemorySize, (int)(kGranMaxB * 128 + 128)));
-    HIP_TRY(hipFuncSetAttribute((const void*)p1_ring_kernel<uint32_t, false, kHashXS, 1, RouteListDirect>, hipFuncAttributeMaxDynamicSharedMemorySize, (int)(kGranMaxB * 128 + 128)));
-    HIP_TRY(hipFuncSetAttribute((const void*)p1_ring_kernel<uint32_t, false, kHashXS, 0, RouteListDirect>, hipFuncAttributeMaxDynamicSharedMemorySize, (int)(kGranMaxB * 128 + 128)));
-    HIP_TRY(hipFuncSetAttribute((const void*)p1_ring_kernel<uint32_t, false, kHashXSLow, 2, RouteListDirect>, hipFuncAttributeMaxDynamicSharedMemorySize, (int)(kGranMaxB * 128 + 128)));
+    HIP_TRY(hipFuncSetAttribute((const void*)p1_ring_kernel<uint32_t, false, 6, 1, RouteListDirect>, hipFuncAttributeMaxDynamicSharedMemorySize, (int)ring_lds_bytes(kGranMaxB)));
+    HIP_TRY(hipFuncSetAttribute((const void*)p1_ring_kernel<uint32_t, false, 6, 0, RouteListDirect>, hipFuncAttributeMaxDynamicSharedMemorySize, (int)ring_lds_bytes(kGranMaxB)));
+    HIP_TRY(hipFuncSetAttribute((const void*)p1_ring_kernel<uint32_t, false, 0, 2, RouteListDirect>, hipFuncAttributeMaxDynamicSharedMemorySize, (int)ring_lds_bytes(kGranMaxB)));
+    HIP_TRY(hipFuncSetAttribute((const void*)p1_ring_kernel<uint32_t, true, 0, 2, RouteListDirect>, hipFuncAttributeMaxDynamicSharedMemorySize, (int)ring_lds_bytes(kGranMaxB)));
+    HIP_TRY(hipFuncSetAttribute((const void*)p1_ring_kernel<uint32_t, false, kHashXS, 1, RouteListDirect>, hipFuncAttributeMaxDynamicSharedMemorySize, (int)ring_lds_bytes(kGranMaxB)));
+    HIP_TRY(hipFuncSetAttribute((const void*)p1_ring_kernel<uint32_t, false, kHashXS, 0, RouteListDirect>, hipFuncAttributeMaxDynamicSharedMemorySize, (int)ring_lds_bytes(kGranMaxB)));
+    HIP_TRY(hipFuncSetAttribute((const void*)p1_ring_kernel<uint32_t, false, kHashXSLow, 2, RouteListDirect>, hipFuncAttributeMaxDynamicSharedMemorySize, (int)ring_lds_bytes(kGranMaxB)));
 #define SATTR(SW) HIP_TRY(hipFuncSetAttribute((const void*)p2_granule_kernel<uint32_t, TableDirect<true>, kP2PairPer, SW>, hipFuncAttributeMaxDynamicSharedMemorySize, kPBlock * kP2PairPer * 4)); \
                   HIP_TRY(hipFuncSetAttribute((const void*)p2_granule_kernel<uint32_t, TableDirect<false>, kP2PairPer, SW>, hipFuncAttributeMaxDynamicSharedMemorySize, kPBlock * kP2PairPer * 4))
     SATTR(1); SATTR(2); SATTR(4);
@@ -816,6 +816,8 @@
               c[0], c[1], c[2], c[3], c[4]);
       fprintf(stderr, "[phase prof] P2: (barrier) %llu  load %llu  hist %llu  scan %llu  lds-scatter %llu  write-out %llu  finish %llu\n",
               c[8], c[9], c[10], c[11], c[12], c[13], c[14]);
+      fprintf(stderr, "[phase prof] P2 (loader / storer rings, the same slots): storers (barrier) %llu  flush %llu | loaders loads+loop %llu  append %llu  (barrier) %llu\n",
+              c[8], c[9], c[10], c[11], c[12]);
       fprintf(stderr, "[phase prof] T: loop+offsets %llu  rank adds + fill %llu  place %llu  merge %llu  queue (wave 0's own) %llu  (its wait for the others) %llu  store %llu\n",
               c[16], c[17], c[18], c[22], c[21], c[19], c[20]);
       (void)hipMemcpyToSymbol(HIP_SYMBOL(g_phase_prof), z, sizeof z);
@@ -1276,7 +1278,8 @@
   rc = read_counters(t, c); if(rc) return rc;
   const uint64_t v[JFGPU_N_COUNTERS] = {c[CTR_FULL], c[CTR_MERS], c[CTR_OVF_FULL], c[CTR_OVF_USED], c[CTR_MISROUTED], c[CTR_DIRECT],
                                         c[CTR_T_ITEMS], c[CTR_T_QUEUED], t->flushes_plain, t->flushes_heavy,
-                                        t->n_p2_roles, t->n_p2_ring, t->n_p2_sort, t->n_p2_exact, t->n_p1_ring, t->n_p1_other};
+                                        t->n_p2_roles, t->n_p2_ring, t->n_p2_sort, t->n_p2_exact, t->n_p1_ring, t->n_p1_other,
+                                        c[CTR_RING_HOLED], c[CTR_RING_STRAG]};
   for(uint32_t i = 0; i < n; ++i) out[i] = i < JFGPU_N_COUNTERS ? v[i] : 0;
   return JFGPU_OK;
 }
diff --git a/jellyfish_amd/csrc/kernels.hip.hpp b/jellyfish_amd/csrc/kernels.hip.hpp
--- a/jellyfish_amd/csrc/kernels.hip.hpp
+++ b/jellyfish_amd/csrc/kernels.hip.hpp
@@ -11,7 +11,9 @@
 
 enum Counter : int { CTR_FULL = 0, CTR_MERS = 1, CTR_OVF_FULL = 2, CTR_OVF_USED = 3, CTR_MISROUTED = 4, CTR_DIRECT = 5,
                      CTR_T_ITEMS = 6, CTR_T_QUEUED = 7 ,
-                     CTR_PROF0 = 8 , CTR_COUNT = 12 };
+                     CTR_PROF0 = 8 ,
+                     CTR_RING_HOLED = 12 ,
+                     CTR_RING_STRAG = 13 , CTR_COUNT = 14 };
 
 #ifdef JFGPU_PHASE_PROF
 __device__ unsigned long long g_phase_prof[24];
@@ -19,14 +21,16 @@
   long long acc[8] = {0, 0, 0, 0, 0, 0, 0, 0}; long long t;
   __device__ PhaseClk() { t = clock64(); }
   __device__ void mark(int i) { const long long n = clock64(); acc[i] += n - t; t = n; }
-  __device__ void flush(int base) { if(threadIdx.x == 0) for(int i = 0; i < 8; ++i) if(acc[i]) atomicAdd(&g_phase_prof[base + i], (unsigned long long)acc[i]); }
+  __device__ void flush(int base, unsigned tid = 0) { if(threadIdx.x == tid) for(int i = 0; i < 8; ++i) if(acc[i]) atomicAdd(&g_phase_prof[base + i], (unsigned long long)acc[i]); }
 };
 #define JF_PHASE(pc, i) (pc).mark(i)
 #define JF_PHASE_FLUSH(pc, base) (pc).flush(base)
+#define JF_PHASE_FLUSH_AT(pc, base, tid) (pc).flush(base, tid)
 #else
 struct PhaseClk {};
 #define JF_PHASE(pc, i) do {} while(0)
 #define JF_PHASE_FLUSH(pc, base) do {} while(0)
+#define JF_PHASE_FLUSH_AT(pc, base, tid) do {} while(0)
 #endif
 
 struct DevBloom {
diff --git a/jellyfish_amd/csrc/kernels_bloom_part.hip.hpp b/jellyfish_amd/csrc/kernels_bloom_part.hip.hpp
--- a/jellyfish_amd/csrc/kernels_bloom_part.hip.hpp
+++ b/jellyfish_amd/csrc/kernels_bloom_part.hip.hpp
@@ -34,6 +34,7 @@
 }
 struct BloomRingDirect {
   uint32_t* data;
+  __device__ unsigned long long* ring_counters() const { return nullptr; }
   __device__ void operator()(uint32_t dest, uint64_t item, uint32_t cnt) const { for(uint32_t i = 0; i < cnt; ++i) bloom_segment_item_direct_call(data, dest, (uint32_t)item); }
 };
 
@@ -165,12 +166,11 @@
                                                                 unsigned int* __restrict__ gcur, unsigned long long* __restrict__ tot,
                                                                 uint32_t* __restrict__ out, unsigned long long* __restrict__ mers,
                                                                 uint64_t* __restrict__ strag, uint32_t* __restrict__ strag_n) {
-  using R = Ring<uint32_t, kBloomRingBytes>;
   JF_DYN_LDS(s_dyn);
   const uint32_t nb = 1u << BP.b1;
   uint32_t* s_ring = reinterpret_cast<uint32_t*>(s_dyn);
-  uint4* s_tn = reinterpret_cast<uint4*>(s_dyn + (size_t)nb * kBloomRingBytes + kBloomRingBytes);
-  __shared__ uint32_t s_fill[kGranMaxB + 32];
+  uint4* s_tn = reinterpret_cast<uint4*>(s_dyn + ring_lds_bytes(nb, kBloomRingBytes));
+  __shared__ uint32_t s_fill[kGranMaxB + kDumpRings];
   __shared__ uint32_t s_nstrag;
   __shared__ uint32_t s_codes[kPBlock + 2];
   __shared__ uint32_t s_inv[kPBlock + 2];
@@ -183,12 +183,12 @@
     s_tn[i] = make_uint4((uint32_t)a, (uint32_t)(a >> 32), (uint32_t)c, (uint32_t)(c >> 32));
   }
   ring_init<uint32_t, kBloomRingBytes>(s_ring, s_fill, nb, &s_nstrag);
-  const uint32_t dump = nb * R::kSlots + (lane & (R::kSlots - 1));
+  const uint32_t spare = nb + (lane & (kDumpRings - 1));
   unsigned int* const gshort = gcur + nb;
   uint64_t* const my_strag = strag + (size_t)blockIdx.x * kStragPerBlock;
   const uint32_t k = g.k, rc_shift = 2 * (k - 1);
   const uint32_t sub_mask = (1u << BP.b2) - 1u;
-  RingBooks Bk;
+  RingBooks Bk = ring_books<uint32_t, kBloomRingBytes>(t);
   if(owner) { Bk.nxt = atomicAdd(&gcur[t], kGran); Bk.nxt_asked = true; }
   uint32_t* const my_region = out + (uint64_t)t * cap;
   uint32_t my_mers = 0;
@@ -233,22 +233,13 @@
           const uint32_t seg = (uint32_t)(byte >> kBloomSegBits);
           const uint32_t b = seg >> BP.b2;
           ei[e] = ((seg & sub_mask) << kBloomItemLow) | ((uint32_t)(byte & 0xFFFFu) << 3) | dig;
-          const uint32_t o = atomicAdd(&s_fill[on ? b : nb + (lane & 31u)], 1u);
-          ea[e] = on ? b * R::kSlots : dump; eo[e] = on ? o : 0u;
+          const uint32_t bs = on ? b : spare;
+          eo[e] = atomicAdd(&s_fill[bs], on ? 4u : 0u);
+          ea[e] = bs * kBloomRingBytes;
           cell += inc; if(cell >= B.m) cell -= B.m;
         }
-        uint32_t ghosts = 0;
-#pragma unroll
-        for(int e = 0; e < PER; ++e) {
-          const uint32_t full = eo[e] & R::kFull;
-          ghosts |= full;
-          const uint32_t at = ea[e] + ((eo[e] + (eo[e] >> 16)) & (R::kSlots - 1));
-          s_ring[full ? dump : at] = ei[e];
-        }
-        if(ghosts) {
-#pragma unroll 1
-          for(int e = 0; e < PER; ++e) if(eo[e] & R::kFull) straggler(ea[e] / R::kSlots, ei[e], 1u);
-        }
+        if(ring_store_round<uint32_t, kBloomRingBytes, PER>(s_ring, ea, eo, ei, spare * kBloomRingBytes))
+          ring_full_entries<uint32_t, kBloomRingBytes, PER>(ea, eo, ei, [&](uint32_t b, uint32_t x) { straggler(b, x, 1u); });
         lds_barrier();
         wave_prio<3>();
         if(owner) ring_flush<uint32_t, false, kBloomRingBytes>(s_ring, s_fill, t, false, Bk, my_region, cap, gcur, gshort, straggler);
diff --git a/jellyfish_amd/csrc/kernels_p1ring.hip.hpp b/jellyfish_amd/csrc/kernels_p1ring.hip.hpp
--- a/jellyfish_amd/csrc/kernels_p1ring.hip.hpp
+++ b/jellyfish_amd/csrc/kernels_p1ring.hip.hpp
@@ -20,14 +20,18 @@
 
 constexpr uint32_t kStragPerBlock = 16384;
 
+constexpr uint32_t kDumpRings = 16;
 template <typename ITEM, uint32_t RB = 128> struct Ring {
   static constexpr uint32_t kSlots = RB / sizeof(ITEM);
   static constexpr uint32_t kUnit = 64 / sizeof(ITEM);
   static constexpr uint32_t kChunk = 16 / sizeof(ITEM);
-  static constexpr uint32_t kFull = 0xFFFFu & ~(kSlots - 1);
   static constexpr uint32_t kWords = sizeof(ITEM) <= 4 ? 1 : 1 + sizeof(ITEM) / 8;
-  __device__ static uint32_t first_fill(uint32_t b) { return ((kChunk * b) & (kSlots - 1)) << 16; }
+  static constexpr uint32_t kFull = 0xFFFFu & ~(RB - 1);
+  __device__ static uint32_t first_head(uint32_t b) { return (16u * b) & (RB - 1); }
+  __device__ static uint32_t first_fill(uint32_t b) { return first_head(b) << 16; }
+  __device__ static uint32_t slot_of(uint32_t o) { return (o + (o >> 16)) & (RB - 1); }
 };
+constexpr size_t ring_lds_bytes(size_t nb, size_t rb = 128) { return (nb + kDumpRings) * rb; }
 
 template <typename ITEM> __device__ __forceinline__ uint32_t chunk_hole_key(const uint4& v) {
   if constexpr(sizeof(ITEM) == 4) { const uint32_t a = v.x > v.y ? v.x : v.y, c = v.z > v.w ? v.z : v.w; return a > c ? a : c; }
@@ -54,28 +58,48 @@
   else item = (ITEM)(((unsigned __int128)rec[2] << 64) | rec[1]);
 }
 
-struct RingBooks { uint32_t gpos = 0, room = 0, nxt = 0, stored = 0; bool nxt_asked = false, exhausted = false; };
+struct RingBooks { uint32_t gpos = 0, room = 0, nxt = 0, stored = 0, head = 0, seen = 0, holed = 0; bool nxt_asked = false, exhausted = false; };
+template <typename ITEM, uint32_t RB = 128> __device__ __forceinline__ RingBooks ring_books(uint32_t t) { RingBooks B; B.head = Ring<ITEM, RB>::first_head(t); return B; }
+
+struct RingPeek { uint32_t w; uint4 v[4]; };
+template <typename ITEM, uint32_t RB = 128>
+__device__ __forceinline__ void ring_peek(const ITEM* s_ring, const uint32_t* s_fill, uint32_t t, const RingBooks& B, RingPeek& P) {
+  const unsigned char* ring = reinterpret_cast<const unsigned char*>(s_ring) + (size_t)t * RB;
+  P.w = s_fill[t];
+#pragma unroll
+  for(int q = 0; q < 4; ++q) P.v[q] = *reinterpret_cast<const uint4*>(ring + ((B.head + 16u * q) & (RB - 1)));
+}
 
 template <typename ITEM, bool OWNED = false, uint32_t RB = 128, typename STRAG>
-__device__ __forceinline__ void ring_flush(ITEM* s_ring, uint32_t* s_fill, uint32_t t, bool all, RingBooks& B, ITEM* my_region, uint32_t cap,
+__device__ __forceinline__ void ring_flush(ITEM* s_ring, uint32_t* s_fill, uint32_t t, bool all, RingBooks& B, const RingPeek& P, ITEM* my_region, uint32_t cap,
                                            unsigned int* gcur, unsigned int* gshort, STRAG&& straggler) {
   using R = Ring<ITEM, RB>;
   const ITEM hole = (ITEM)~(ITEM)0;
-  const uint32_t w = s_fill[t];
-  uint32_t cnt = w & 0xFFFFu; if(cnt > R::kSlots) cnt = R::kSlots;
-  const uint32_t rb = (w >> 16) & (R::kSlots - 1);
-  uint32_t units = cnt / R::kUnit; if(all && (cnt % R::kUnit)) ++units;
+  unsigned char* const ring = reinterpret_cast<unsigned char*>(s_ring) + (size_t)t * RB;
+  const uint32_t cnt = P.w & 0xFFFFu;
+  const uint32_t win = cnt < RB ? cnt : RB;
+  uint32_t units = win / 64; if(all && (win % 64)) ++units;
   uint32_t nout = 0;
   for(uint32_t s = 0; s < units; ++s) {
     uint4 v[4];
-    const uint32_t s0 = (rb + s * R::kUnit) & (R::kSlots - 1);
-#pragma unroll
-    for(int q = 0; q < 4; ++q) v[q] = *reinterpret_cast<const uint4*>(s_ring + t * R::kSlots + ((s0 + R::kChunk * q) & (R::kSlots - 1)));
-    if(!all) {
-      uint32_t mx = 0;
-#pragma unroll
-      for(int q = 0; q < 4; ++q) { const uint32_t a = chunk_hole_key<ITEM>(v[q]); mx = mx > a ? mx : a; }
-      if(mx == 0xFFFFFFFFu) break;
+    const uint32_t s0 = (B.head + s * 64) & (RB - 1);
+    if(s == 0) {
+#pragma unroll
+      for(int q = 0; q < 4; ++q) v[q] = P.v[q];
+    } else {
+#pragma unroll
+      for(int q = 0; q < 4; ++q) v[q] = *reinterpret_cast<const uint4*>(ring + ((s0 + 16u * q) & (RB - 1)));
+    }
+    uint32_t mx = 0;
+#pragma unroll
+    for(int q = 0; q < 4; ++q) { const uint32_t a = chunk_hole_key<ITEM>(v[q]); mx = mx > a ? mx : a; }
+    uint32_t real = R::kUnit;
+    if(mx == 0xFFFFFFFFu) {
+      if(!all && (s + 1) * 64 > B.seen) break;
+      real = 0;
+#pragma unroll
+      for(int q = 0; q < 4; ++q) chunk_items<ITEM>(v[q], [&](ITEM x) { real += x != hole ? 1u : 0u; });
+      if(!all) ++B.holed;
     }
     if constexpr(!OWNED) {
     if(B.room == 0 && B.nxt_asked) {
@@ -93,7 +117,6 @@
       uint4* dst = reinterpret_cast<uint4*>(my_region + B.gpos);
 #pragma unroll
       for(int q = 0; q < 4; ++q) dst[q] = v[q];
-      const uint32_t real = cnt - s * R::kUnit < R::kUnit ? cnt - s * R::kUnit : R::kUnit;
       B.gpos += R::kUnit; B.room -= R::kUnit; B.stored += real;
     } else {
 #pragma unroll
@@ -101,28 +124,65 @@
     }
 #pragma unroll
     for(int q = 0; q < 4; ++q)
-      *reinterpret_cast<uint4*>(s_ring + t * R::kSlots + ((s0 + R::kChunk * q) & (R::kSlots - 1))) = make_uint4(0xFFFFFFFFu, 0xFFFFFFFFu, 0xFFFFFFFFu, 0xFFFFFFFFu);
+      *reinterpret_cast<uint4*>(ring + ((s0 + 16u * q) & (RB - 1))) = make_uint4(0xFFFFFFFFu, 0xFFFFFFFFu, 0xFFFFFFFFu, 0xFFFFFFFFu);
     ++nout;
   }
   if constexpr(!OWNED) { if(!all && !B.nxt_asked && !B.exhausted && B.room < R::kSlots) { B.nxt = atomicAdd(&gcur[t], kGran); B.nxt_asked = true; } }
-  uint32_t expect = w;
-  while(nout || (expect & 0xFFFFu) > R::kSlots) {
-    uint32_t c = expect & 0xFFFFu; if(c > R::kSlots) c = R::kSlots;
-    const uint32_t taken = nout * R::kUnit < c ? nout * R::kUnit : c;
-    const uint32_t neww = ((((expect >> 16) + nout * R::kUnit) & 0xFFFFu) << 16) | (c - taken);
-    const uint32_t old = atomicCAS(&s_fill[t], expect, neww);
-    if(old == expect) break;
-    expect = old;
-  }
+  const uint32_t moved = nout * 64;
+  const uint32_t taken = (moved < win ? moved : win) + (cnt - win);
+  if(moved | taken) atomicAdd(&s_fill[t], (moved << 16) - taken);
+  B.head = (B.head + moved) & (RB - 1);
+  B.seen = win - (moved < win ? moved : win);
+}
+template <typename ITEM, bool OWNED = false, uint32_t RB = 128, typename STRAG>
+__device__ __forceinline__ void ring_flush(ITEM* s_ring, uint32_t* s_fill, uint32_t t, bool all, RingBooks& B, ITEM* my_region, uint32_t cap,
+                                           unsigned int* gcur, unsigned int* gshort, STRAG&& straggler) {
+  RingPeek P;
+  ring_peek<ITEM, RB>(s_ring, s_fill, t, B, P);
+  ring_flush<ITEM, OWNED, RB>(s_ring, s_fill, t, all, B, P, my_region, cap, gcur, gshort, straggler);
 }
 
 template <typename ITEM, uint32_t RB = 128>
 __device__ __forceinline__ void ring_init(ITEM* s_ring, uint32_t* s_fill, uint32_t nb, uint32_t* s_nstrag) {
   using R = Ring<ITEM, RB>;
-  for(uint32_t j = threadIdx.x; j < nb; j += blockDim.x) s_fill[j] = R::first_fill(j);
+  for(uint32_t j = threadIdx.x; j < nb + kDumpRings; j += blockDim.x) s_fill[j] = j < nb ? R::first_fill(j) : 0u;
   uint4* r4 = reinterpret_cast<uint4*>(s_ring);
-  for(uint32_t j = threadIdx.x; j < nb * (RB / 16) + RB / 16; j += blockDim.x) r4[j] = make_uint4(0xFFFFFFFFu, 0xFFFFFFFFu, 0xFFFFFFFFu, 0xFFFFFFFFu);
+  for(uint32_t j = threadIdx.x; j < (nb + kDumpRings) * (RB / 16); j += blockDim.x) r4[j] = make_uint4(0xFFFFFFFFu, 0xFFFFFFFFu, 0xFFFFFFFFu, 0xFFFFFFFFu);
   if(threadIdx.x == 0) *s_nstrag = 0;
+}
+
+template <typename ITEM, uint32_t RB, int NE>
+__device__ __forceinline__ bool ring_store_round(ITEM* s_ring, const uint32_t (&ea)[NE], const uint32_t (&eo)[NE], const ITEM (&ei)[NE], uint32_t dump_at) {
+  using R = Ring<ITEM, RB>;
+  unsigned char* const ring = reinterpret_cast<unsigned char*>(s_ring);
+  uint32_t any = 0;
+#pragma unroll
+  for(int e = 0; e < NE; ++e) any |= eo[e];
+  if(!(any & R::kFull)) {
+#pragma unroll
+    for(int e = 0; e < NE; ++e) *reinterpret_cast<ITEM*>(ring + (ea[e] | R::slot_of(eo[e]))) = ei[e];
+    return false;
+  }
+#pragma unroll
+  for(int e = 0; e < NE; ++e) *reinterpret_cast<ITEM*>(ring + ((eo[e] & R::kFull) ? dump_at : (ea[e] | R::slot_of(eo[e])))) = ei[e];
+  return true;
+}
+
+template <typename ITEM, uint32_t RB, int NE, typename F>
+__device__ __forceinline__ void ring_full_entries(const uint32_t (&ea)[NE], const uint32_t (&eo)[NE], const ITEM (&ei)[NE], F&& f) {
+#pragma unroll 1
+  for(int e = 0; e < NE; ++e) {
+    uint32_t a = 0, o = 0; ITEM it = 0;
+#pragma unroll
+    for(int q = 0; q < NE; ++q) if(q == e) { a = ea[q]; o = eo[q]; it = ei[q]; }
+    if(o & Ring<ITEM, RB>::kFull) f(a / RB, it);
+  }
+}
+
+__device__ __forceinline__ void ring_count_events(unsigned long long* counters, uint32_t holed, uint32_t stragglers) {
+  if(!counters) return;
+  if(holed) atomicAdd(&counters[CTR_RING_HOLED], (unsigned long long)holed);
+  if(stragglers) atomicAdd(&counters[CTR_RING_STRAG], (unsigned long long)stragglers);
 }
 
 template <typename ITEM>
@@ -161,7 +221,7 @@
   JF_DYN_LDS(s_dyn);
   ITEM* s_ring = reinterpret_cast<ITEM*>(s_dyn);
   __shared__ uint64_t s_fwd[NB < 0 ? 1 : 8 * 256];
-  __shared__ uint32_t s_fill[kGranMaxB + 32];
+  __shared__ uint32_t s_fill[kGranMaxB + kDumpRings];
   __shared__ uint32_t s_nstrag;
   __shared__ uint32_t s_codes[kPBlock + 2];
   __shared__ uint32_t s_inv[kPBlock + 2];
@@ -172,14 +232,14 @@
   const ITEM hole = (ITEM)~(ITEM)0;
   if constexpr(NB >= 0) load_tables_lds(s_fwd, T.fwd_tbl, g.nbytes);
   ring_init<ITEM>(s_ring, s_fill, nb, &s_nstrag);
-  const uint32_t dump = nb * R::kSlots + (lane & (R::kSlots - 1));
+  const uint32_t spare = nb + (lane & (kDumpRings - 1));
   [[maybe_unused]] const uint32_t xs_hi_mask = g.lsize_g > 32 ? (g.lsize_g >= 64 ? 0xFFFFFFFFu : ((1u << (g.lsize_g - 32)) - 1u)) : 0u;
   unsigned int* const gshort = gcur + nb;
   uint64_t* const my_strag = strag + (size_t)blockIdx.x * kStragPerBlock * R::kWords;
   const uint32_t k = g.k, bshift = g.lsize_l - P.b1;
   const uint32_t rc_shift = 2 * (k - 1);
   const uint32_t rest_mask = P.rest_shift >= 32 ? 0xFFFFFFFFu : ((1u << P.rest_shift) - 1u);
-  RingBooks B;
+  RingBooks B = ring_books<ITEM>(t);
   if(owner) { B.nxt = atomicAdd(&gcur[t], kGran); B.nxt_asked = true; }
   ITEM* const my_region = out + (uint64_t)t * cap;
   uint32_t my_mers = 0, my_direct = 0;
@@ -213,9 +273,9 @@
     for(int j0 = 0; j0 < kPerLane; j0 += RP) {
       constexpr int NE = RUNS ? RP + 1 : RP;
       uint32_t ea[NE], eo[NE]; ITEM ei[NE];
-      [[maybe_unused]] uint32_t spm = 0;
-#pragma unroll
-      for(int e = 0; e < NE; ++e) { ea[e] = dump; ei[e] = 0; eo[e] = 0; }
+      if constexpr(RUNS) { ea[NE - 1] = spare * 128u; eo[NE - 1] = 0; ei[NE - 1] = 0; }
+      constexpr bool FOLD = !RUNS && sizeof(ITEM) == 4;
+      [[maybe_unused]] uint32_t hmax = 0;
       auto emit = [&](int e, uint64_t key, uint32_t cnt, bool on) {
         uint32_t b; ITEM item;
         if constexpr(NB == kHashXS && sizeof(ITEM) == 4) {
@@ -229,17 +289,16 @@
           if constexpr(sizeof(ITEM) == 4) item = (((uint32_t)pos & rest_mask) << g.rem_bits) | (uint32_t)(key >> g.lsize_g);
           else item = make_item<ITEM>(g, P, key, pos & g.local_mask);
         }
-        const bool special = on && (item == hole || cnt > 1);
-        const bool normal = on && !special;
-#ifndef JFGPU_P1_LATE_SPECIAL
-        if(special) straggler(b, item, cnt);
-        const uint32_t o = atomicAdd(&s_fill[normal ? b : nb + (lane & 31u)], 1u);
-        ea[e] = normal ? b * R::kSlots : dump; ei[e] = item; eo[e] = normal ? o : 0u;
-#else
-        const uint32_t o = atomicAdd(&s_fill[normal ? b : nb + (lane & 31u)], 1u);
-        spm |= special ? 1u << e : 0u;
-        ea[e] = on ? b * R::kSlots : dump; ei[e] = item; eo[e] = normal ? o : special ? (R::kFull | ((cnt < 0xFFFFu ? cnt : 0xFFFFu) << 16)) : 0u;
-#endif
+        bool normal = on;
+        if constexpr(FOLD) { const uint32_t x = (uint32_t)item; hmax = hmax > x ? hmax : x; }
+        else {
+          const bool special = on && (item == hole || cnt > 1);
+          normal = on && !special;
+          if(special) straggler(b, item, cnt);
+        }
+        const uint32_t bs = normal ? b : spare;
+        eo[e] = atomicAdd(&s_fill[bs], normal ? (uint32_t)sizeof(ITEM) : 0u);
+        ea[e] = bs * (uint32_t)(R::kSlots * sizeof(ITEM)); ei[e] = item;
       };
 #ifndef JFGPU_P1_OLD_EXTRACT
       const uint32_t cur_r = L.cur << (2 * j0), ncur_r = ~cur_r, vm_r = vmask << j0;
@@ -275,26 +334,18 @@
         } else emit(e, key, 1u, v != 0);
       }
       if constexpr(RUNS) { if(j0 + RP >= kPerLane) { emit(NE - 1, pk, run, pv != 0); pv = 0; } }
-      uint32_t ghosts = 0;
-#pragma unroll
-      for(int e = 0; e < NE; ++e) {
-        const uint32_t full = eo[e] & R::kFull;
-        ghosts |= full;
-        const uint32_t at = ea[e] + ((eo[e] + (eo[e] >> 16)) & (R::kSlots - 1));
-        s_ring[full ? dump : at] = ei[e];
-      }
-      if(ghosts) {
-#pragma unroll 1
-#ifndef JFGPU_P1_LATE_SPECIAL
-        for(int e = 0; e < NE; ++e) {
-          uint32_t a = 0, o = 0; ITEM it = 0;
-#pragma unroll
-          for(int q = 0; q < NE; ++q) if(q == e) { a = ea[q]; o = eo[q]; it = ei[q]; }
-          if(o & R::kFull) straggler(a / R::kSlots, it, 1u);
-        }
-#else
-        for(int e = 0; e < NE; ++e) if(eo[e] & R::kFull) straggler(ea[e] / R::kSlots, ei[e], ((spm >> e) & 1u) ? eo[e] >> 16 : 1u);
-#endif
+      if(ring_store_round<ITEM, 128, NE>(s_ring, ea, eo, ei, spare * 128u))
+        ring_full_entries<ITEM, 128, NE>(ea, eo, ei, [&](uint32_t b, ITEM it) { straggler(b, it, 1u); });
+      if constexpr(FOLD) {
+        if(hmax == 0xFFFFFFFFu) {
+#pragma unroll 1
+          for(int e = 0; e < NE; ++e) {
+            uint32_t a = 0; ITEM it = 0;
+#pragma unroll
+            for(int q = 0; q < NE; ++q) if(q == e) { a = ea[q]; it = ei[q]; }
+            if(it == hole && a < nb * 128u) straggler(a / 128u, it, 1u);
+          }
+        }
       }
       JF_PHASE(pc, 1);
       lds_barrier();
@@ -323,6 +374,7 @@
   if(owner) { ring_flush<ITEM>(s_ring, s_fill, t, true, B, my_region, cap, gcur, gshort, straggler); ring_finish<ITEM>(B, t, my_region, cap, gshort, tot); }
   lds_barrier();
   if(t == 0) strag_n[blockIdx.x] = s_nstrag < kStragPerBlock ? s_nstrag : kStragPerBlock;
+  ring_count_events((unsigned long long*)T.counters, B.holed, t == 0 ? s_nstrag : 0u);
   JF_PHASE(pc, 4);
   JF_PHASE_FLUSH(pc, 0);
   if(DIRECT::kCountsDirect && my_direct) atomicAdd((unsigned long long*)&T.counters[CTR_DIRECT], (unsigned long long)my_direct);
@@ -359,6 +411,7 @@
 
 struct P2RingDirect {
   const DevTable* Tm; uint32_t b2; uint32_t dest_shift; int returning;
+  __device__ unsigned long long* ring_counters() const { return (unsigned long long*)Tm->counters; }
   __device__ void operator()(uint32_t dest, uint64_t item, uint32_t cnt) const { item_direct_call(Tm, b2, dest >> dest_shift, item, cnt, returning); }
 };
 
@@ -367,11 +420,10 @@
                                                           unsigned int* __restrict__ gcur, unsigned int* __restrict__ gshort,
                                                           uint32_t* __restrict__ out, uint32_t bucket0, unsigned long long* __restrict__ tot,
                                                           uint64_t* __restrict__ strag, uint32_t* __restrict__ strag_n, unsigned long long* __restrict__ ctr_direct) {
-  using R = Ring<uint32_t>;
   constexpr int RP = 8;
   JF_DYN_LDS(s_dyn);
   uint32_t* s_ring = reinterpret_cast<uint32_t*>(s_dyn);
-  __shared__ uint32_t s_fill[kGranMaxB];
+  __shared__ uint32_t s_fill[kGranMaxB + kDumpRings];
   __shared__ uint32_t s_nstrag;
   const uint32_t nb = 1u << b2e;
   const uint32_t bucket = bucket0 + blockIdx.y;
@@ -380,12 +432,12 @@
   const bool owner = t < nb;
   const uint32_t hole = 0xFFFFFFFFu;
   ring_init<uint32_t>(s_ring, s_fill, nb, &s_nstrag);
-  const uint32_t dump = nb * R::kSlots + (lane & (R::kSlots - 1));
+  const uint32_t spare = nb + (lane & (kDumpRings - 1));
   unsigned int* const gc = gcur + dest0;
   unsigned int* const gs = gshort + dest0;
   const uint32_t list = blockIdx.y * gridDim.x + blockIdx.x;
   uint64_t* const my_strag = strag + (size_t)list * kP2StragPerBlock;
-  RingBooks B;
+  RingBooks B = ring_books<uint32_t>(t);
   if(owner) { B.nxt = atomicAdd(&gc[t], kGran); B.nxt_asked = true; }
   uint32_t* const my_region = out + ((uint64_t)dest0 + t) * cap;
   uint32_t my_direct = 0;
@@ -433,21 +485,13 @@
     uint32_t ea[RP], eo[RP];
 #pragma unroll
     for(int e = 0; e < RP; ++e) {
-      ea[e] = dump; eo[e] = 0;
-      if(it[e] != hole) { const uint32_t d = (it[e] >> tag_bits) & (nb - 1); ea[e] = d * R::kSlots; eo[e] = atomicAdd(&s_fill[d], 1u); }
-    }
-    uint32_t ghosts = 0;
-#pragma unroll
-    for(int e = 0; e < RP; ++e) {
-      const uint32_t full = eo[e] & R::kFull;
-      ghosts |= full;
-      const uint32_t at = ea[e] + ((eo[e] + (eo[e] >> 16)) & (R::kSlots - 1));
-      s_ring[full ? dump : at] = it[e];
-    }
-    if(ghosts) {
-#pragma unroll 1
-      for(int e = 0; e < RP; ++e) if(eo[e] & R::kFull) straggler(ea[e] / R::kSlots, it[e], 1u);
-    }
+      const bool real = it[e] != hole;
+      const uint32_t bs = real ? (it[e] >> tag_bits) & (nb - 1) : spare;
+      eo[e] = atomicAdd(&s_fill[bs], real ? 4u : 0u);
+      ea[e] = bs * 128u;
+    }
+    if(ring_store_round<uint32_t, 128, RP>(s_ring, ea, eo, it, spare * 128u))
+      ring_full_entries<uint32_t, 128, RP>(ea, eo, it, [&](uint32_t d, uint32_t x) { straggler(d, x, 1u); });
     lds_barrier();
     flush(false);
     lds_barrier();
@@ -475,6 +519,7 @@
   if(owner) ring_finish<uint32_t>(B, t, my_region, cap, gs, tot ? tot + dest0 : nullptr);
   lds_barrier();
   if(t == 0) strag_n[list] = s_nstrag < kP2StragPerBlock ? s_nstrag : kP2StragPerBlock;
+  ring_count_events(D.ring_counters(), B.holed, t == 0 ? s_nstrag : 0u);
   if(my_direct) atomicAdd(ctr_direct, (unsigned long long)my_direct);
 }
 
@@ -489,7 +534,7 @@
   constexpr uint64_t RS = (uint64_t)kHalf * RP;
   JF_DYN_LDS(s_dyn);
   ITEM* s_ring = reinterpret_cast<ITEM*>(s_dyn);
-  __shared__ uint32_t s_fill[kGranMaxB];
+  __shared__ uint32_t s_fill[kGranMaxB + kDumpRings];
   __shared__ uint32_t s_nstrag;
   const uint32_t nb = 1u << b2e;
   const uint32_t bucket = bucket0 + blockIdx.x;
@@ -498,37 +543,43 @@
   const bool storer = t < kHalf;
   const ITEM hole = (ITEM)~(ITEM)0;
   ring_init<ITEM>(s_ring, s_fill, nb, &s_nstrag);
-  const uint32_t dump = nb * R::kSlots + (lane & (R::kSlots - 1));
+  const uint32_t spare = nb + (lane & (kDumpRings - 1));
   uint64_t* const my_strag = strag + (size_t)blockIdx.x * kP2StragPerBlock * R::kWords;
-  uint32_t my_direct = 0;
+  uint32_t my_direct = 0, my_holed = 0;
   auto straggler = [&](uint32_t d, ITEM item, uint32_t cnt) {
     const uint32_t at = atomicAdd(&s_nstrag, 1u);
     if(at < kP2StragPerBlock) strag_store<ITEM>(my_strag + (size_t)at * R::kWords, dest0 + d, item, cnt);
     else { D(dest0 + d, item, cnt); ++my_direct; }
   };
   lds_barrier();
+  [[maybe_unused]] PhaseClk pc;
   auto seg_bounds = [&](uint32_t seg, uint64_t& a, uint64_t& b) { a = seg_lo(S, seg, bucket); b = seg_hi(S, seg, bucket); };
   if(storer) {
     const uint32_t d0 = t, d1 = t + kHalf;
     const bool has0 = d0 < nb, has1 = d1 < nb;
-    RingBooks B0, B1;
+    RingBooks B0 = ring_books<ITEM>(d0), B1 = ring_books<ITEM>(d1);
     B0.room = B1.room = cap & ~(R::kUnit - 1);
     ITEM* const r0p = out + ((uint64_t)dest0 + d0) * cap;
     ITEM* const r1p = out + ((uint64_t)dest0 + d1) * cap;
     auto flush = [&](bool all) {
-      if(has0) ring_flush<ITEM, true>(s_ring, s_fill, d0, all, B0, r0p, cap, gcur, gcur, straggler);
-      if(has1) ring_flush<ITEM, true>(s_ring, s_fill, d1, all, B1, r1p, cap, gcur, gcur, straggler);
+      RingPeek P0, P1;
+      ring_peek<ITEM>(s_ring, s_fill, has0 ? d0 : 0u, B0, P0);
+      ring_peek<ITEM>(s_ring, s_fill, has1 ? d1 : 0u, B1, P1);
+      if(has0) ring_flush<ITEM, true>(s_ring, s_fill, d0, all, B0, P0, r0p, cap, gcur, gcur, straggler);
+      if(has1) ring_flush<ITEM, true>(s_ring, s_fill, d1, all, B1, P1, r1p, cap, gcur, gcur, straggler);
     };
     for(uint32_t seg = 0; seg < S.n; ++seg) {
       uint64_t a, b; seg_bounds(seg, a, b);
       const uint64_t rounds = (b - a + RS - 1) / RS;
 #pragma unroll 1
-      for(uint64_t r = 0; r < rounds; ++r) { lds_barrier(); flush(false); }
+      for(uint64_t r = 0; r < rounds; ++r) { lds_barrier(); JF_PHASE(pc, 0); flush(false); JF_PHASE(pc, 1); }
     }
     lds_barrier();
     flush(true);
+    JF_PHASE_FLUSH(pc, 8);
     if(has0) gcur[dest0 + d0] = B0.gpos;
     if(has1) gcur[dest0 + d1] = B1.gpos;
+    my_holed = B0.holed + B1.holed;
   } else {
     const uint32_t l = t - kHalf;
     for(uint32_t seg = 0; seg < S.n; ++seg) {
@@ -563,25 +614,20 @@
         }
       };
       auto append = [&](const ITEM (&it)[RP]) {
+        JF_PHASE(pc, 2);
         uint32_t ea[RP], eo[RP];
 #pragma unroll
         for(int e = 0; e < RP; ++e) {
-          ea[e] = dump; eo[e] = 0;
-          if(it[e] != hole) { const uint32_t d = (uint32_t)(it[e] >> tag_bits) & (nb - 1); ea[e] = d * R::kSlots; eo[e] = atomicAdd(&s_fill[d], 1u); }
-        }
-        uint32_t ghosts = 0;
-#pragma unroll
-        for(int e = 0; e < RP; ++e) {
-          const uint32_t full = eo[e] & R::kFull;
-          ghosts |= full;
-          const uint32_t at = ea[e] + ((eo[e] + (eo[e] >> 16)) & (R::kSlots - 1));
-          s_ring[full ? dump : at] = it[e];
-        }
-        if(ghosts) {
-#pragma unroll 1
-          for(int e = 0; e < RP; ++e) if(eo[e] & R::kFull) straggler(ea[e] / R::kSlots, it[e], 1u);
-        }
+          const bool real = it[e] != hole;
+          const uint32_t bs = real ? (uint32_t)(it[e] >> tag_bits) & (nb - 1) : spare;
+          eo[e] = atomicAdd(&s_fill[bs], real ? (uint32_t)sizeof(ITEM) : 0u);
+          ea[e] = bs * 128u;
+        }
+        if(ring_store_round<ITEM, 128, RP>(s_ring, ea, eo, it, spare * 128u))
+          ring_full_entries<ITEM, 128, RP>(ea, eo, it, [&](uint32_t d, ITEM x) { straggler(d, x, 1u); });
+        JF_PHASE(pc, 3);
         lds_barrier();
+        JF_PHASE(pc, 4);
       };
       uint64_t r0 = a;
       if(S.sh[seg] == 0) {
@@ -615,9 +661,11 @@
       if(r0 < b) { ITEM it[RP]; load_partial(r0, it); append(it); }
     }
     lds_barrier();
+    JF_PHASE_FLUSH_AT(pc, 8, kHalf);
   }
   lds_barrier();
   if(t == 0) strag_n[blockIdx.x] = s_nstrag < kP2StragPerBlock ? s_nstrag : kP2StragPerBlock;
+  ring_count_events(D.ring_counters(), my_holed, t == 0 ? s_nstrag : 0u);
   if(my_direct) atomicAdd(ctr_direct, (unsigned long long)my_direct);
 }
 
```

Result: no change. 15.33 billion (median of 2 runs) (+0.8%).
